# cherise215/Cooperative_Training_and_Latent_Space_Data_Augmentation

Measured on AMD Instinct MI355X. Metric: cooperative-training slices/sec (256x256, bs16 per GPU), higher is better.
Workload: dtype f32 (bf16x3 split)

## Files before the change

cooperative_training_and_latent_space_data_augmentation_amd/_ffi.py:

```python
from __future__ import annotations

import ctypes as C
import os

import numpy as np

_HERE = os.path.dirname(os.path.abspath(__file__))
LIB_PATH = os.path.join(_HERE, "csrc", "libctl_hip.so")
ABI_VERSION = 11
RED_BLOCKS = 512

IN_PLAIN, IN_UP2, IN_ZINS2, IN_C4 = 0, 1, 2, 3
ACT_NONE, ACT_LEAKY, ACT_SIGMOID = 0, 1, 2
EPI_BIAS, EPI_ACCUM, EPI_RES, EPI_STATS, EPI_BNBWD, EPI_TAILBWD = 1, 2, 4, 8, 16, 32
(OP_CONV, OP_WGRAD, OP_WGRAD_REDUCE, OP_PACK, OP_BN_FINALIZE, OP_BN_EVAL, OP_BN_ACT, OP_BWD_REDUCE, OP_BN_BWD_FINALIZE,
 OP_BWD_APPLY, OP_CHAN_SUM_FINALIZE, OP_SUMPOOL2, OP_SIGMOID_BWD, OP_ZERO, OP_COPY, OP_PACK_BATCH, OP_WGRAD_REDUCE_BATCH, OP_DROPOUT2D, OP_BN_REPLAY,
 OP_WGRAD_GROUP) = range(1, 21)
WGRAD_GROUP_MAX = 8
OP_MAX_T = 14

CONV_DTYPE = np.dtype([
    ("n", "<i4"), ("hin", "<i4"), ("win", "<i4"), ("cin", "<i4"), ("hout", "<i4"), ("wout", "<i4"), ("cout", "<i4"),
    ("ks", "<i4"), ("stride", "<i4"), ("pad", "<i4"), ("in_mode", "<i4"), ("pro_affine", "<i4"), ("pro_slope", "<f4"),
    ("epi_flags", "<i4"), ("epi_act", "<i4"), ("epi_slope", "<f4"), ("out_h", "<i4"), ("out_w", "<i4"),
    ("out_sy", "<i4"), ("out_sx", "<i4"), ("nsub", "<i4"), ("out_sub", "<i4"), ("groups", "<i4"), ("dt", "<i4")])
DT_BF16, DT_X16, DT_Y16, DT_RES16, DT_X3 = 1, 2, 4, 8, 16
PACK_X3 = 16
LOSS_WCE, LOSS_FOCAL, LOSS_DICE, LOSS_FG_DICE = 0, 1, 2, 3
OP_DTYPE = np.dtype([("kind", "<i4"), ("i", "<i4", (27,)), ("f", "<f4", (4,)), ("slot", "<i4", (OP_MAX_T,)),
                     ("off", "<i8", (OP_MAX_T,)), ("l", "<i8", (4,))], align=True)


class CtlError(RuntimeError):
    pass


class _Lib:
    def __init__(self):
        self._lib = None

    def load(self):
        if self._lib is not None:
            return self._lib
        if not os.path.exists(LIB_PATH):
            raise CtlError(f"HIP extension not built: {LIB_PATH} is missing. Run `python -c 'import __graft_entry__ as g; "
                           "g.build()'` (or `make -C <package>/csrc`). There is no fallback path.")
        import torch
        lib = C.CDLL(LIB_PATH)
        lib.ctl_last_error.restype = C.c_char_p
        lib.ctl_version.restype = C.c_int
        lib.ctl_launch_count.restype = C.c_ulonglong
        for name in ("ctl_conv_wpack_floats", "ctl_conv_stats_floats", "ctl_wgrad_partial_floats",
                     "ctl_wgrad_bias_partial_floats", "ctl_latent_score_ws_floats", "ctl_latent_mask_apply_ws_floats",
                     "ctl_rescale_intensity_ws_floats", "ctl_sizeof_op", "ctl_sizeof_conv", "ctl_latent_mask_fused_ws_floats", "ctl_conv_wpack_floats_x3",
                     "ctl_surface_stats_ws_bytes", "ctl_surface_map_ws_bytes", "ctl_cc_ws_bytes", "ctl_aug_ws_bytes", "ctl_aug_warp_ws_bytes",
                     "ctl_surface_quantiles_ws_bytes",
                     "ctl_aug_spline_ws_bytes", "ctl_aug_warp_cubic_ws_bytes", "ctl_aug_bias_ws_bytes", "ctl_order_stats_ws_bytes", "ctl_corrupt_spike_ws_bytes",
                     "ctl_seg_loss_ws_doubles"):
            getattr(lib, name).restype = C.c_size_t
        p, i32, i64, f32, u64 = C.c_void_p, C.c_int32, C.c_int64, C.c_float, C.c_uint64
        sig = {
            "ctl_conv_wpack_floats": [i32, i32, i32],
            "ctl_conv_stats_floats": [p], "ctl_conv_stats_blocks": [p],
            "ctl_wgrad_splits": [p], "ctl_wgrad_partial_floats": [p], "ctl_wgrad_bias_partial_floats": [p],
            "ctl_pack_weights": [p, p, i32, i32, i32, i64, i64, i64, i64, i32, p],
            "ctl_conv_forward": [p] * 12, "ctl_conv_forward_ex": [p] * 16, "ctl_conv_pool_ok": [p],
            "ctl_conv_wgrad": [p] * 8, "ctl_conv_wgrad_ex": [p] * 10,
            "ctl_wgrad_group_class": [p, i32], "ctl_wgrad_group_plan": [p, i32, p], "ctl_conv_wgrad_group": [i32] + [p] * 11,
            "ctl_wgrad_reduce": [p, p, p, p, i64, i64, i64, i64, p, i32, p],
            "ctl_confusion_hist": [p, p, i64, i32, p, p],
            "ctl_rescale_intensity": [p, p, p, i32, i64, f32, f32, f32, p],
            "ctl_noise_clamp": [p, p, u64, f32, f32, f32, p, i64, p],
            "ctl_rescale_intensity_ws_floats": [i32],
            "ctl_crop_or_pad": [p, p, i32, i32, i32, i32, i32, i32, p],
            "ctl_bn_finalize": [p, i32, i32, i64, p, p, f32, f32, i32, p, p, p, p, p, p, p, i32, p],
            "ctl_bn_finalize_ex": [p, i32, i32, i64, p, p, f32, f32, i32, p, p, p, p, p, p, p, p, i32, p],
            "ctl_bn_replay_running": [p, p, p, p, i32, f32, p],
            "ctl_bn_eval_coeffs": [i32, p, p, p, p, f32, p, p, i32, p],
            "ctl_bn_act": [p, p, p, f32, p, i64, i32, i32, p],
            "ctl_bwd_reduce": [i32, p, p, p, p, p, f32, i64, i32, p, i32, p], "ctl_red_blocks": [],
            "ctl_bn_bwd_finalize": [p, i32, i64, p, p, p, p, p, p, i32, i32, i32, p],
            "ctl_bn_bwd_finalize_ex": [p, i32, i64, p, p, p, p, p, p, i32, i32, i32, C.c_uint32, p],
            "ctl_bwd_apply": [i32, p, p, p, p, p, f32, p, i64, i32, p, p, i32, p],
            "ctl_chan_sum_finalize": [p, i32, p, i32, p],
            "ctl_sumpool2": [p, p, i32, i32, i32, i32, i32, p],
            "ctl_sigmoid_bwd": [p, p, p, i64, p],
            "ctl_softmax_t_fwd": [p, f32, p, i64, i32, p],
            "ctl_softmax_t_bwd": [p, p, f32, p, i64, i32, p],
            "ctl_onehot": [p, p, i64, i32, p],
            "ctl_ce2d_fwd": [p, p, i64, i32, p, p, p],
            "ctl_ce2d_bwd": [p, p, p, i64, i32, p, p],
            "ctl_mse_fwd": [p, p, i64, f32, p, p, p],
            "ctl_mse_bwd": [p, p, p, i64, f32, p, p],
            "ctl_argmax_c": [p, p, i64, i32, p],
            "ctl_latent_score_ws_floats": [i32, i32, i32, i32],
            "ctl_latent_score": [i32, p, p, p, i32, i32, i32, p],
            "ctl_latent_mask_apply": [i32, p, p, p, i32, p, p, p, p, i32, i32, i32, p],
            "ctl_latent_mask_apply_ws_floats": [i32, i32, i32, i32],
            "ctl_latent_mask_fused_ws_floats": [i32, i32, i32, i32],
            "ctl_latent_mask_fused": [i32, p, p, p, i32, p, p, p, p, p, i32, i32, i32, p],
            "ctl_dropout2d": [p, p, u64, f32, p, p, i32, i32, i32, p],
            "ctl_uniform": [p, i64, u64, p],
            "ctl_step_tick": [p, p],
            "ctl_spin": [i32, p],
            "ctl_dropout2d_ex": [p, p, u64, p, f32, p, p, p, i32, i32, i32, p],
            "ctl_dropout2d_dt": [p, p, u64, p, f32, p, p, i32, i32, i32, C.c_uint32, p],
            "ctl_uniform_dev": [p, i64, u64, p, p],
            "ctl_adam_dev": [p, p, p, p, i64, f32, f32, f32, f32, p, f32, p],
            "ctl_adam": [p, p, p, p, i64, f32, f32, f32, f32, i32, f32, p],
            "ctl_accumulate": [p, p, i32, i64, p],
            "ctl_plan_run": [p, i32, p, i32, p],
            "ctl_prof_start": [C.c_char_p], "ctl_prof_start_sampled": [C.c_char_p, i32], "ctl_prof_stop": [p, C.c_size_t],
            "ctl_pack_weights_batched": [p, p, p, i32, i64, p], "ctl_wgrad_reduce_batched": [p, p, p, i32, i64, p],
            "ctl_pack_weights_bf16_batched": [p, p, p, i32, i64, p],
            "ctl_pack_weights_x3_batched": [p, p, p, i32, i64, p], "ctl_conv_wpack_floats_x3": [i32, i32, i32],
            "ctl_bwd_reduce_rows": [i32, i64, i32],
            "ctl_bn_act_dt": [p, p, p, f32, p, i64, i32, i32, C.c_uint32, p],
            "ctl_bwd_reduce_dt": [i32, p, p, p, p, p, f32, i64, i32, p, i32, C.c_uint32, p, p],
            "ctl_bwd_apply_dt": [i32, p, p, p, p, p, f32, p, i64, i32, p, p, i32, C.c_uint32, p],
            "ctl_sumpool2_dt": [p, p, i32, i32, i32, i32, i32, C.c_uint32, p],
            "ctl_surface_stats_rows": [i32, i32, i32, i32], "ctl_surface_stats_ws_bytes": [i32] * 6,
            "ctl_surface_stats": [p, p, i32, i32, i32, i32, i32, i32, i32, p, p, p, C.c_size_t, p],
            "ctl_surface_map_ws_bytes": [i32] * 4,
            "ctl_surface_quantiles_ws_bytes": [i32] * 7,
            "ctl_surface_quantiles": [p, p, i32, i32, i32, i32, i32, i32, i32, p, p, i32, p, p, p, C.c_size_t, p],
            "ctl_surface_map": [p, i32, i32, i32, i32, i32, p, p, p, p, C.c_size_t, p],
            "ctl_cc_ws_bytes": [i32] * 5, "ctl_cc_label": [p, i32, i32, i32, i32, i32, i32, p, p],
            "ctl_cc_keep_largest": [p, i32, i32, i32, i32, i32, i32, p, p, p, C.c_size_t, p],
            "ctl_aug_ws_bytes": [i32] * 3, "ctl_aug_warp_ws_bytes": [i32] * 5, "ctl_aug_field": [p, p, p, p, i32, i32, i32, p, p, C.c_size_t, p],
            "ctl_aug_warp": [p, p, p, p, p, i32, i32, i32, i32, i32, p, p, p, C.c_size_t, p],
            "ctl_aug_spline_ws_bytes": [i32] * 4, "ctl_aug_warp_cubic_ws_bytes": [i32] * 6,
            "ctl_aug_spline_coeffs": [p, p, p, i32, i32, i32, i32, p, p, C.c_size_t, p],
            "ctl_aug_warp_cubic": [p, p, p, p, p, i32, i32, i32, i32, i32, i32, p, p, p, C.c_size_t, p],
            "ctl_aug_bias_ws_bytes": [i32] * 3, "ctl_aug_bias": [p, p, p, p, i32, i32, i32, p, p, C.c_size_t, p],
            "ctl_aug_coarse_field": [p, i32, i32, i32, p, p],
            "ctl_order_stats_ws_bytes": [i32, i32], "ctl_order_stats": [p, i32, i64, p, i32, p, p, C.c_size_t, p],
            "ctl_percentile_apply": [p, p, i32, i64, C.c_double, C.c_double, i32, f32, f32, p, p, p],
            "ctl_resample_inplane": [p, p, i32, i32, i32, i32, i32, i32, C.c_double, C.c_double, p, p, p],
            "ctl_restore_scores": [p, i32, i32, i32, i32, i32, i32, i32, i32, i32, i32, C.c_double, C.c_double, i32, p, p, p],
            "ctl_restore_labels": [p, i32, i32, i32, i32, i32, i32, i32, i32, i32, C.c_double, C.c_double, p, p],
            "ctl_corrupt_bias": [p, p, i32, i32, i32, p, p], "ctl_corrupt_spike_ws_bytes": [i32] * 4,
            "ctl_corrupt_spike": [p, i32, i32, i32, p, p, i32, C.c_double, p, p, C.c_size_t, p],
            "ctl_corrupt_rigid3d": [p, i32, i32, i32, p, i32, p, p], "ctl_axis_operator": [p, p, i32, i32, i32, i32, i32, p, p, p],
            "ctl_slice_foreground": [p, p, i32, i64, p, p],
            "ctl_batch_gather": [p, p, p, i32, i64, p, i32, p, i32, i32, p, p, i32, i32, p, p, p],
            "ctl_seg_loss_blocks": [i32, i64], "ctl_seg_loss_ws_doubles": [i32, i32, i64, i32],
            "ctl_seg_loss_fwd": [i32, p, p, p, f32, i32, i64, i32, p, p, p],
            "ctl_seg_loss_bwd": [i32, p, p, p, f32, p, p, i32, i64, i32, p, p],
        }
        for name, args in sig.items():
            getattr(lib, name).argtypes = args
        if lib.ctl_version() != ABI_VERSION or lib.ctl_sizeof_op() != OP_DTYPE.itemsize or lib.ctl_sizeof_conv() != CONV_DTYPE.itemsize:
            raise CtlError(f"ABI mismatch: library version {lib.ctl_version()} vs binding {ABI_VERSION}, sizeof(ctl_op)={lib.ctl_sizeof_op()} "
                           f"vs {OP_DTYPE.itemsize}, sizeof(ctl_conv)={lib.ctl_sizeof_conv()} vs {CONV_DTYPE.itemsize}")
        if lib.ctl_red_blocks() != RED_BLOCKS:
            raise CtlError(f"ABI mismatch: the library was built with CTL_RED_BLOCKS={lib.ctl_red_blocks()}, this binding sizes scratch for {RED_BLOCKS}")
        self._lib = lib
        return lib

    def __getattr__(self, name):
        return getattr(self.load(), name)


lib = _Lib()

EXPORTED = ["ctl_version", "ctl_last_error", "ctl_conv_wpack_floats", "ctl_conv_stats_floats", "ctl_conv_stats_blocks",
            "ctl_pack_weights", "ctl_conv_forward", "ctl_conv_forward_ex", "ctl_conv_pool_ok", "ctl_wgrad_splits", "ctl_wgrad_partial_floats",
            "ctl_wgrad_bias_partial_floats", "ctl_conv_wgrad", "ctl_conv_wgrad_ex", "ctl_wgrad_reduce", "ctl_bn_finalize", "ctl_bn_finalize_ex", "ctl_bn_replay_running", "ctl_bn_eval_coeffs",
            "ctl_bn_act", "ctl_bwd_reduce", "ctl_bn_bwd_finalize", "ctl_bn_bwd_finalize_ex", "ctl_bwd_apply", "ctl_chan_sum_finalize", "ctl_sumpool2",
            "ctl_sigmoid_bwd", "ctl_softmax_t_fwd", "ctl_softmax_t_bwd", "ctl_onehot", "ctl_ce2d_fwd", "ctl_ce2d_bwd",
            "ctl_mse_fwd", "ctl_mse_bwd", "ctl_argmax_c", "ctl_latent_score_ws_floats", "ctl_latent_score",
            "ctl_latent_mask_apply", "ctl_latent_mask_apply_ws_floats", "ctl_dropout2d", "ctl_uniform", "ctl_adam", "ctl_plan_run", "ctl_sizeof_op",
            "ctl_sizeof_conv", "ctl_prof_start", "ctl_prof_start_sampled", "ctl_prof_stop", "ctl_pack_weights_batched",
            "ctl_wgrad_reduce_batched", "ctl_confusion_hist", "ctl_rescale_intensity_ws_floats", "ctl_rescale_intensity",
            "ctl_noise_clamp", "ctl_crop_or_pad", "ctl_step_tick", "ctl_spin", "ctl_dropout2d_ex", "ctl_dropout2d_dt", "ctl_uniform_dev", "ctl_adam_dev",
            "ctl_latent_mask_fused_ws_floats", "ctl_latent_mask_fused", "ctl_accumulate", "ctl_pack_weights_bf16_batched",
            "ctl_bn_act_dt", "ctl_bwd_reduce_dt", "ctl_bwd_apply_dt", "ctl_sumpool2_dt", "ctl_bwd_reduce_rows", "ctl_red_blocks",
            "ctl_launch_count", "ctl_conv_wpack_floats_x3", "ctl_pack_weights_x3_batched", "ctl_wgrad_group_class", "ctl_wgrad_group_plan",
            "ctl_conv_wgrad_group", "ctl_surface_stats_rows", "ctl_surface_stats_ws_bytes", "ctl_surface_stats", "ctl_surface_map_ws_bytes",
            "ctl_surface_map", "ctl_cc_ws_bytes", "ctl_cc_label", "ctl_cc_keep_largest", "ctl_aug_ws_bytes", "ctl_aug_warp_ws_bytes", "ctl_aug_field",
            "ctl_aug_warp", "ctl_aug_spline_ws_bytes", "ctl_aug_warp_cubic_ws_bytes", "ctl_aug_spline_coeffs", "ctl_aug_warp_cubic",
            "ctl_aug_bias_ws_bytes", "ctl_aug_bias", "ctl_aug_coarse_field", "ctl_order_stats_ws_bytes", "ctl_order_stats",
            "ctl_percentile_apply", "ctl_resample_inplane", "ctl_corrupt_bias", "ctl_corrupt_spike_ws_bytes", "ctl_corrupt_spike",
            "ctl_corrupt_rigid3d", "ctl_axis_operator", "ctl_slice_foreground", "ctl_batch_gather", "ctl_surface_quantiles_ws_bytes",
            "ctl_surface_quantiles", "ctl_restore_scores", "ctl_restore_labels", "ctl_seg_loss_blocks", "ctl_seg_loss_ws_doubles",
            "ctl_seg_loss_fwd", "ctl_seg_loss_bwd"]


def prof_start(kernel_filter: str = "", every: int = 1) -> None:
    check(lib.ctl_prof_start_sampled(kernel_filter.encode(), int(every)), "ctl_prof_start_sampled")


def prof_stop() -> dict:
    buf = C.create_string_buffer(1 << 18)
    check(lib.ctl_prof_stop(buf, len(buf)), "ctl_prof_stop")
    out = {}
    for line in buf.value.decode().splitlines():
        parts = line.split()
        out[parts[0]] = {k: float(v) for k, v in (kv.split("=") for kv in parts[1:])}
    return out


def check(rc: int, what: str = "") -> None:
    if rc != 0:
        msg = lib.ctl_last_error()
        raise CtlError(f"{what} failed (rc={rc}): {msg.decode() if msg else ''}")


def conv_desc(**kw) -> np.ndarray:
    d = np.zeros((), dtype=CONV_DTYPE)
    d["pad"] = 1 if kw.get("ks", 3) in (3, 4) else 0
    d["stride"] = 1
    d["nsub"] = 1
    d["groups"] = 1
    d["out_sy"] = d["out_sx"] = 1
    for k, v in kw.items():
        d[k] = v
    if "out_h" not in kw:
        d["out_h"] = d["hout"]
    if "out_w" not in kw:
        d["out_w"] = d["wout"]
    return d


def desc_ptr(d: np.ndarray) -> int:
    return d.ctypes.data
```

cooperative_training_and_latent_space_data_augmentation_amd/csrc/ctl_conv.hip:

```cpp
#include <stdlib.h>

#include <type_traits>

#include "ctl_common.h"

#include "ctl_conv_common.h"

#ifdef CTL_TIMING
#define CTL_TM_WAVES 65536
__device__ unsigned long long ctl_tm[CTL_TM_WAVES][10];
#define TM_DECL unsigned long long tm_prev = __builtin_amdgcn_s_memtime(), tm_acc[10] = {0, 0, 0, 0, 0, 0, 0, 0, 0, 0}; \
                const unsigned long long tm_t0 = tm_prev, tm_r0 = __builtin_amdgcn_s_memrealtime();
#define TM(i) { const unsigned long long tm_now = __builtin_amdgcn_s_memtime(); tm_acc[i] += tm_now - tm_prev; tm_prev = tm_now; }
#define TM_COUNT(i) { tm_acc[i] += 1; }
#define TM_FLUSH { const unsigned w_ = ((blockIdx.x + gridDim.x * (blockIdx.y + gridDim.y * blockIdx.z)) * 4 + (threadIdx.x >> 6)) % CTL_TM_WAVES; \
                   tm_acc[8] = __builtin_amdgcn_s_memtime() - tm_t0; tm_acc[9] = __builtin_amdgcn_s_memrealtime() - tm_r0; \
                   if ((threadIdx.x & 63) == 0) { _Pragma("unroll") for (int i_ = 0; i_ < 10; ++i_) ctl_tm[w_][i_] += tm_acc[i_]; } }
extern "C" int ctl_debug_timing(unsigned long long* out8) {
    static unsigned long long host[CTL_TM_WAVES][10];
    if (hipMemcpyFromSymbol(host, HIP_SYMBOL(ctl_tm), sizeof(host)) != hipSuccess) return -1;
    for (int i = 0; i < 12; ++i) out8[i] = 0;
    for (int w = 0; w < CTL_TM_WAVES; ++w) {
        for (int i = 0; i < 10; ++i) out8[i] += host[w][i];
        if (host[w][8] > out8[10]) out8[10] = host[w][8];
// ... 540 lines not shown
    const bool is_w = idx < total;
    const bool is_b = !is_w && dbias != nullptr && idx < total + cout;
    float v = 0.f;
    int co = 0, ci = 0, tap = 0;
    if (is_w) {
        co = idx % cout;
        ci = (idx / cout) % cin;
        tap = idx / ((int64_t)cout * cin);
        const int64_t stride = (int64_t)taps * cin_p * cout_p;
        const float* src = w_partial + ((int64_t)tap * cin_p + ci) * cout_p + co;
        for (int s = sl; s < splits; s += 8) v += src[s * stride];
    } else if (is_b) {
        co = idx - total;
        for (int s = sl; s < splits; s += 8) v += b_partial[(int64_t)s * cout_p + co];
    }
    sm[sl][e] = v;
    __syncthreads();
    if (sl == 0 && (is_w || is_b)) {
        float t = 0.f;
#pragma unroll
        for (int k = 0; k < 8; ++k) t += sm[k][e];
        float* dst = is_w ? dw + co * s_co + ci * s_ci + (tap / ks) * s_kh + (tap % ks) * s_kw : dbias + co;
        *dst = accumulate ? (*dst + t) : t;
    }
}

__global__ void pack_weights_kernel(const float* __restrict__ src, float* __restrict__ dst, int cout, int cin, int ks,
                                    int g_chunks, int64_t total, int64_t s_co, int64_t s_ci, int64_t s_kh,
                                    int64_t s_kw, int flip) {
    const int64_t idx = (int64_t)blockIdx.x * blockDim.x + threadIdx.x;
    if (idx >= total) return;
    const int j = idx & 3, lane = (idx >> 2) & 63;
    int64_t rest = idx >> 8;
    const int g = rest % g_chunks;
    rest /= g_chunks;
    const int taps = ks * ks;
    const int tap = rest % taps;
    const int cot = rest / taps;
    const int co = cot * 16 + (lane & 15);
    const int ci = g * 16 + (lane >> 4) * 4 + j;
    int kh = tap / ks, kw = tap % ks;
    if (flip) { kh = ks - 1 - kh; kw = ks - 1 - kw; }
    float v = 0.f;
    if (co < cout && ci < cin) v = src[co * s_co + ci * s_ci + kh * s_kh + kw * s_kw];
    dst[idx] = v;
}

__global__ void pack_weights_batched_kernel(const float* __restrict__ params, float* __restrict__ wpack,
                                            const int64_t* __restrict__ table) {
    const int64_t* r = table + (int64_t)blockIdx.y * 12;
    const int64_t total = r[10];
    const int64_t idx = (int64_t)blockIdx.x * blockDim.x + threadIdx.x;
    if (idx >= total || (r[11] & CTL_PACK_X3)) return;
    const float* src = params + r[0];
    float* dst = wpack + r[1];
    const int cout = (int)r[2], cin = (int)r[3], ks = (int)r[4], flip = (int)r[5];
    const int g_chunks = (cin + 15) / 16;
    const int j = idx & 3, lane = (idx >> 2) & 63;
    int64_t rest = idx >> 8;
    const int g = rest % g_chunks;
    rest /= g_chunks;
    const int taps = ks * ks;
    const int tap = rest % taps;
    const int cot = rest / taps;
    const int co = cot * 16 + (lane & 15);
    const int ci = g * 16 + (lane >> 4) * 4 + j;
    int kh = tap / ks, kw = tap % ks;
    float v = 0.f;
    if (r[11] == 4) {
        const int c = j, quad = (int)((idx >> 8) % 3), cot4 = (int)((idx >> 8) / 3);
        const int co4 = cot4 * 16 + (lane & 15), tp = 4 * quad + (lane >> 4);
        if (co4 < cout && c < cin && tp < 9) v = src[co4 * r[6] + c * r[7] + (tp / 3) * r[8] + (tp % 3) * r[9]];
        dst[idx] = v;
        return;
    }
    if (r[11] == 1) {
        if (co < cout && ci < cin) {
            for (int a = 0; a < 2; ++a) {
                const int sh = a + 2 - kh;
                if (sh < 0 || sh > 2) continue;
                for (int b = 0; b < 2; ++b) {
                    const int sw = b + 2 - kw;
                    if (sw < 0 || sw > 2) continue;
                    v += src[co * r[6] + ci * r[7] + sh * r[8] + sw * r[9]];
                }
            }
        }
    } else if (r[11] == 2) {
        if (co < cout && ci < cin) {
            const int a = flip >> 1, b = flip & 1;
            const int h0 = (kh == 0) ? 0 : (a ? 2 : 1), h1 = (kh == 0) ? (a ? 1 : 0) : 2;
            const int w0 = (kw == 0) ? 0 : (b ? 2 : 1), w1 = (kw == 0) ? (b ? 1 : 0) : 2;
            for (int sh = h0; sh <= h1; ++sh)
                for (int sw = w0; sw <= w1; ++sw) v += src[co * r[6] + ci * r[7] + sh * r[8] + sw * r[9]];
        }
    } else if (r[11] == 3) {
        if (co < cout && ci < cin) {
            const int a = flip >> 1, b = flip & 1;
            const int sh = a ? (kh == 0 ? 2 : 0) : (kh == 0 ? 1 : -1);
            const int sw = b ? (kw == 0 ? 2 : 0) : (kw == 0 ? 1 : -1);
            if (sh >= 0 && sw >= 0) v = src[co * r[6] + ci * r[7] + sh * r[8] + sw * r[9]];
        }
    } else {
        if (flip) { kh = ks - 1 - kh; kw = ks - 1 - kw; }
        if (co < cout && ci < cin) v = src[co * r[6] + ci * r[7] + kh * r[8] + kw * r[9]];
    }
    dst[idx] = v;
}

__global__ __launch_bounds__(256) void wgrad_reduce_batched_kernel(const float* __restrict__ scratch, float* __restrict__ grad,
                                                                    const int64_t* __restrict__ table) {
    __shared__ float sm[32][65];
    const int64_t* r = table + (int64_t)blockIdx.y * 16;
    const int splits = (int)r[4], taps = (int)(r[5] & 0xff), ks = (int)(r[5] >> 8), cin = (int)r[6], cout = (int)r[7];
    const int cin_p = (int)r[8], cout_p = (int)r[9];
    const int64_t total = (int64_t)taps * cin * cout;
    const bool has_b = r[1] >= 0 && r[3] >= 0;
    const bool wide = splits <= 64;
    const int EW = wide ? 64 : 8, SLN = wide ? 4 : 32;
    if ((int64_t)blockIdx.x * EW >= total + (has_b ? cout : 0)) return;
    const int e = wide ? (threadIdx.x & 63) : (threadIdx.x & 7), sl = wide ? (threadIdx.x >> 6) : (threadIdx.x >> 3);
    const int64_t idx = (int64_t)blockIdx.x * EW + e;
    const bool is_w = idx < total, is_b = !is_w && has_b && idx < total + cout;
    float v = 0.f;
    int co = 0, ci = 0, tap = 0;
    if (is_w) {
        co = idx % cout;
        ci = (idx / cout) % cin;
        tap = idx / ((int64_t)cout * cin);
        const int64_t stride = (int64_t)taps * cin_p * cout_p;
        const float* src = scratch + r[0] + ((int64_t)tap * cin_p + ci) * cout_p + co;
        for (int s0 = sl; s0 < splits; s0 += 8 * SLN) {
            float t8[8];
#pragma unroll
            for (int u = 0; u < 8; ++u) { const int s = s0 + u * SLN; t8[u] = s < splits ? src[s * stride] : 0.f; }
#pragma unroll
            for (int u = 0; u < 8; ++u) v += t8[u];
        }
    } else if (is_b) {
        co = idx - total;
        const float* src = scratch + r[1] + co;
        for (int s = sl; s < splits; s += SLN) v += src[(int64_t)s * cout_p];
    }
    sm[sl][e] = v;
    __syncthreads();
    if (sl == 0 && (is_w || is_b)) {
        float t = 0.f;
        for (int k = 0; k < SLN; ++k) t += sm[k][e];
        float* dst = is_w ? grad + r[2] + co * r[10] + ci * r[11] + (tap / ks) * r[12] + (tap % ks) * r[13] : grad + r[3] + co;
        *dst = r[14] ? (*dst + t) : t;
    }
}

extern "C" int ctl_pack_weights_batched(const float* params, float* wpack, const int64_t* table, int32_t n_rec,
                                        int64_t max_total, ctl_stream stream) {
    CTL_REQUIRE(params && wpack && table && n_rec > 0 && max_total > 0, "pack_weights_batched: bad arguments");
    pack_weights_batched_kernel<<<dim3((unsigned)ctl_cdiv64(max_total, 256), (unsigned)n_rec), dim3(256), 0, (hipStream_t)stream>>>(
        params, wpack, table);
    CTL_LAUNCH_CHECK("pack_weights_batched");
    return CTL_OK;
}
extern "C" int ctl_wgrad_reduce_batched(const float* scratch, float* grad, const int64_t* table, int32_t n_rec,
                                        int64_t max_elems, ctl_stream stream) {
    CTL_REQUIRE(scratch && grad && table && n_rec > 0 && max_elems > 0, "wgrad_reduce_batched: bad arguments");
    wgrad_reduce_batched_kernel<<<dim3((unsigned)max_elems, (unsigned)n_rec), dim3(256), 0, (hipStream_t)stream>>>(
        scratch, grad, table);
    CTL_LAUNCH_CHECK("wgrad_reduce_batched");
    return CTL_OK;
}

extern "C" size_t ctl_conv_wpack_floats(int32_t cin, int32_t cout, int32_t ks) {
    return (size_t)ctl_cdiv(cout, 16) * ks * ks * ctl_cdiv(cin, 16) * 256;
}

static bool conv_combo_ok(const ctl_conv* d) {
    const int k = d->ks, s = d->stride, m = d->in_mode, pd = d->pad;
    if (k == 3 && s == 1 && pd == 1 && m != CTL_IN_C4) return true;
    if (k == 3 && s == 1 && pd == 1 && m == CTL_IN_C4 && d->cin <= 4 && d->nsub == 1) return true;
    if (k == 3 && s == 2 && pd == 1 && m == CTL_IN_PLAIN) return true;
    if (k == 1 && s == 1 && pd == 0 && m != CTL_IN_ZINS2) return true;
    if (k == 2 && s == 2 && pd == 0 && m == CTL_IN_PLAIN) return true;
    if (k == 4 && s == 2 && pd == 1 && m == CTL_IN_PLAIN) return true;
    if (k == 2 && s == 1 && (pd == 0 || pd == 2) && m == CTL_IN_PLAIN && d->nsub == 4) return true;
    return false;
}

int ctl_conv_pick_cfg(const ctl_conv* d, ctl_conv_cfg* c, int for_wgrad) {
    CTL_REQUIRE(conv_combo_ok(d), "conv: unsupported ks/stride/pad/in_mode %d/%d/%d/%d", d->ks, d->stride, d->pad,
                d->in_mode);
    CTL_REQUIRE(d->cin == 1 || d->cin % 4 == 0, "conv: cin must be 1 or a multiple of 4 (got %d)", d->cin);
    CTL_REQUIRE(d->cout == 1 || d->cout % 4 == 0, "conv: cout must be 1 or a multiple of 4 (got %d)", d->cout);
    CTL_REQUIRE(d->cin < 16 ? (d->cin == 1 || d->cin == 4 || d->cin == 8 || d->cin == 12) : d->cin % 16 == 0,
                "conv: cin >= 16 must be a multiple of 16 (got %d)", d->cin);
    CTL_REQUIRE(d->nsub == 1 || d->nsub == 4, "conv: nsub must be 1 or 4");
    c->cot = ctl_cdiv(d->cout, 16);
    c->g = ctl_cdiv(d->cin, 16);
    c->nt = (c->cot % 2 == 0) ? 2 : 1;
    auto blocks = [&](int mt, int tw) {
        const int th = 4 * mt * 16 / tw;
        return (int64_t)d->n * ctl_cdiv(d->hout, th) * ctl_cdiv(d->wout, tw) * (c->cot / c->nt) * d->nsub;
    };
    int mt, tw;
    if (for_wgrad) {
        if (d->hout >= 8) { mt = 2; tw = 16; }
        else { mt = 1; tw = 16; }
    } else if (d->stride == 2) {
        if (blocks(2, 16) >= 384) { mt = 2; tw = 16; } else { mt = 1; tw = 16; }
        if (d->ks == 4 && c->nt == 2) { mt = 1; tw = 16; }
    } else if (d->wout >= 32 && blocks(4, 32) >= 512 && !(c->nt == 2 && blocks(4, 32) > 768)) {
        mt = 4; tw = 32;
    } else if (blocks(2, 16) >= 384) {
        mt = 2; tw = 16;
// ... 390 lines not shown
```

cooperative_training_and_latent_space_data_augmentation_amd/csrc/ctl_conv_common.h:

```cpp
#pragma once
#include "ctl_common.h"

template <int KS, int S, int MT, int TW>
struct Geom {
    static constexpr int MTILES = 4 * MT;
    static constexpr int TH = MTILES * 16 / TW;
    static constexpr int TP = TH * TW;
    static constexpr int IH = (TH - 1) * S + KS;
    static constexpr int IW = (TW - 1) * S + KS;
    static constexpr int IWH = (IW + 1) / 2;
    static constexpr int IWP = (S == 2) ? 2 * IWH : IW;
    static constexpr int XT_IMAGE = IH * IWP * 16;
    static constexpr int XT_FLOATS = XT_IMAGE + 4;
    static constexpr int PAD = (KS >= 3) ? 1 : 0;
    __device__ static __forceinline__ int ldscol(int c) { return (S == 2) ? ((c & 1) * IWH + (c >> 1)) : c; }
};

typedef unsigned int u32x4 __attribute__((ext_vector_type(4)));
#define CTL_OOB ((int)0x80000000)
#define CTL_PRO_MAX 256

__device__ __forceinline__ __amdgpu_buffer_rsrc_t ctl_rsrc(const void* p, int64_t bytes) {
    return __builtin_amdgcn_make_buffer_rsrc(const_cast<void*>(p), 0, (int)bytes, 0x00020000);
}
__device__ __forceinline__ f32x4 ctl_bload4(__amdgpu_buffer_rsrc_t r, int voff) {
    return __builtin_bit_cast(f32x4, __builtin_amdgcn_raw_buffer_load_b128(r, voff, 0, 0));
}
__device__ __forceinline__ float ctl_bload1(__amdgpu_buffer_rsrc_t r, int voff) {
    return __builtin_bit_cast(float, __builtin_amdgcn_raw_buffer_load_b32(r, voff, 0, 0));
}
#ifndef CTL_STORE_AUX
#define CTL_STORE_AUX 0
#endif
__device__ __forceinline__ void ctl_bstore4(__amdgpu_buffer_rsrc_t r, int voff, f32x4 v) {
    __builtin_amdgcn_raw_buffer_store_b128(__builtin_bit_cast(u32x4, v), r, voff, 0, CTL_STORE_AUX);
}
__device__ __forceinline__ void ctl_bstore1(__amdgpu_buffer_rsrc_t r, int voff, float v) {
    __builtin_amdgcn_raw_buffer_store_b32(__builtin_bit_cast(unsigned int, v), r, voff, 0, 0);
}
__device__ __forceinline__ f32x4 ctl_bload4s(__amdgpu_buffer_rsrc_t r, int voff, int soff) {
    return __builtin_bit_cast(f32x4, __builtin_amdgcn_raw_buffer_load_b128(r, voff, soff, 0));
}
__device__ __forceinline__ f32x4 ctl_leaky01(f32x4 v, float slope) {
    const f32x4 m = v * slope;
    return f32x4{fmaxf(v.x, m.x), fmaxf(v.y, m.y), fmaxf(v.z, m.z), fmaxf(v.w, m.w)};
}

struct TileWalk {
    int n, th, tw;
    int dn, dth, dtw;
    int tiles_h, tiles_w;
    __device__ __forceinline__ void init(int bid0, int nblk, int tiles_h_, int tiles_w_) {
        tiles_h = tiles_h_; tiles_w = tiles_w_;
        tw = bid0 % tiles_w; int b = bid0 / tiles_w; th = b % tiles_h; n = b / tiles_h;
        dtw = nblk % tiles_w; b = nblk / tiles_w; dth = b % tiles_h; dn = b / tiles_h;
    }
    __device__ __forceinline__ void next() {
        tw += dtw;
        if (tw >= tiles_w) { tw -= tiles_w; ++th; }
        th += dth;
        if (th >= tiles_h) { th -= tiles_h; ++n; }
        n += dn;
    }
};
```

cooperative_training_and_latent_space_data_augmentation_amd/csrc/ctl_conv_x3.hip:

```cpp
#include "ctl_common.h"
#ifdef CTL_TIMING_X3
#define CTL_TM_WAVES 65536
__device__ unsigned long long ctl_tm3[CTL_TM_WAVES][10];
#define TM_DECL unsigned long long tm_prev = __builtin_amdgcn_s_memtime(), tm_acc[10] = {0, 0, 0, 0, 0, 0, 0, 0, 0, 0}; \
                const unsigned long long tm_t0 = tm_prev, tm_r0 = __builtin_amdgcn_s_memrealtime();
#define TM(i) { const unsigned long long tm_now = __builtin_amdgcn_s_memtime(); tm_acc[i] += tm_now - tm_prev; tm_prev = tm_now; }
#define TM_COUNT(i) { tm_acc[i] += 1; }
#ifdef CTL_TIMING_X3_VMCNT
#define CTL_TM3_REAL
#else
#define CTL_TM3_REAL tm_acc[9] = __builtin_amdgcn_s_memrealtime() - tm_r0;
#endif
#define TM_FLUSH { const unsigned w_ = ((blockIdx.x + gridDim.x * (blockIdx.y + gridDim.y * blockIdx.z)) * 8 + (threadIdx.x >> 6)) % CTL_TM_WAVES; \
                   tm_acc[8] = __builtin_amdgcn_s_memtime() - tm_t0; CTL_TM3_REAL \
                   if ((threadIdx.x & 63) == 0) { _Pragma("unroll") for (int i_ = 0; i_ < 10; ++i_) ctl_tm3[w_][i_] += tm_acc[i_]; } }
extern "C" int ctl_debug_timing_x3(unsigned long long* out12) {
    static unsigned long long host[CTL_TM_WAVES][10];
    if (hipMemcpyFromSymbol(host, HIP_SYMBOL(ctl_tm3), sizeof(host)) != hipSuccess) return -1;
    for (int i = 0; i < 12; ++i) out12[i] = 0;
    for (int w = 0; w < CTL_TM_WAVES; ++w) {
        for (int i = 0; i < 10; ++i) out12[i] += host[w][i];
        if (host[w][8] > out12[10]) out12[10] = host[w][8];
        if (host[w][8]) out12[11] += 1;
    }
    for (int w = 0; w < CTL_TM_WAVES; ++w) for (int i = 0; i < 10; ++i) host[w][i] = 0;
    return hipMemcpyToSymbol(HIP_SYMBOL(ctl_tm3), host, sizeof(host)) == hipSuccess ? 0 : -1;
}
#endif
#include "ctl_conv_igemm.h"

__device__ static float x3_pack_value(const float* __restrict__ src, const int64_t* __restrict__ r, int mode, int co, int ci, int kh, int kw) {
    const int cout = (int)r[2], cin = (int)r[3], ks = (int)r[4], flip = (int)r[5];
    if (co >= cout || ci >= cin) return 0.f;
    float v = 0.f;
    if (mode == 1) {
        for (int a = 0; a < 2; ++a) {
            const int sh = a + 2 - kh;
            if (sh < 0 || sh > 2) continue;
            for (int b = 0; b < 2; ++b) {
                const int sw = b + 2 - kw;
                if (sw < 0 || sw > 2) continue;
                v += src[co * r[6] + ci * r[7] + sh * r[8] + sw * r[9]];
            }
        }
    } else if (mode == 2) {
        const int a = flip >> 1, b = flip & 1;
        const int h0 = (kh == 0) ? 0 : (a ? 2 : 1), h1 = (kh == 0) ? (a ? 1 : 0) : 2;
        const int w0 = (kw == 0) ? 0 : (b ? 2 : 1), w1 = (kw == 0) ? (b ? 1 : 0) : 2;
        for (int sh = h0; sh <= h1; ++sh)
            for (int sw = w0; sw <= w1; ++sw) v += src[co * r[6] + ci * r[7] + sh * r[8] + sw * r[9]];
    } else if (mode == 3) {
        const int a = flip >> 1, b = flip & 1;
        const int sh = a ? (kh == 0 ? 2 : 0) : (kh == 0 ? 1 : -1);
        const int sw = b ? (kw == 0 ? 2 : 0) : (kw == 0 ? 1 : -1);
        if (sh >= 0 && sw >= 0) v = src[co * r[6] + ci * r[7] + sh * r[8] + sw * r[9]];
    } else {
        if (flip) { kh = ks - 1 - kh; kw = ks - 1 - kw; }
        v = src[co * r[6] + ci * r[7] + kh * r[8] + kw * r[9]];
    }
    return v;
}
__global__ void pack_weights_x3_batched_kernel(const float* __restrict__ params, float* __restrict__ wpack, const int64_t* __restrict__ table) {
    const int64_t* r = table + (int64_t)blockIdx.y * 12;
    if (!(r[11] & CTL_PACK_X3)) return;
    const int mode = (int)(r[11] & ~(int64_t)CTL_PACK_X3);
    const int cout = (int)r[2], cin = (int)r[3], ks = (int)r[4];
    const int g_chunks = (cin + 15) / 16, taps = ks * ks, nfrag = (taps + 1) / 2;
    const int64_t total = (int64_t)((cout + 15) / 16) * nfrag * g_chunks * 64 * 4;
    const int64_t idx = (int64_t)blockIdx.x * blockDim.x + threadIdx.x;
    if (idx >= total) return;
    const float* src = params + r[0];
    unsigned* dst = reinterpret_cast<unsigned*>(wpack + r[1]);
    const int jp = idx & 3, lane = (idx >> 2) & 63;
    int64_t rest = idx >> 8;
    const int g = rest % g_chunks;
    rest /= g_chunks;
    const int f = rest % nfrag;
    const int cot = rest / nfrag;
    const int co = cot * 16 + (lane & 15), q = lane >> 4;
    const int tap = 2 * f + (q >> 1);
    float a = 0.f, b = 0.f;
    if (tap < taps) {
        const int ci = g * 16 + (q & 1) * 8 + jp * 2;
        a = x3_pack_value(src, r, mode, co, ci, tap / ks, tap % ks);
        b = x3_pack_value(src, r, mode, co, ci + 1, tap / ks, tap % ks);
    }
    const int64_t base = ((((int64_t)cot * nfrag + f) * g_chunks + g) * 3) * 256 + lane * 4 + jp;
#pragma unroll
    for (int sp = 0; sp < 3; ++sp) dst[base + sp * 256] = x3_pack2(x3_part(a, sp), x3_part(b, sp));
}
extern "C" size_t ctl_conv_wpack_floats_x3(int32_t cin, int32_t cout, int32_t ks) {
    return (size_t)ctl_cdiv(cout, 16) * ((ks * ks + 1) / 2) * ctl_cdiv(cin, 16) * 3 * 256;
}
extern "C" int ctl_pack_weights_x3_batched(const float* params, float* wpack, const int64_t* table, int32_t n_rec, int64_t max_total, ctl_stream stream) {
    CTL_REQUIRE(params && wpack && table && n_rec > 0 && max_total > 0, "pack_weights_x3_batched: bad arguments");
    pack_weights_x3_batched_kernel<<<dim3((unsigned)ctl_cdiv64(max_total, 3 * 256) + 1, (unsigned)n_rec), dim3(256), 0, (hipStream_t)stream>>>(params, wpack, table);
    CTL_LAUNCH_CHECK("pack_weights_x3_batched");
    return CTL_OK;
}

struct conv3_call {
    const ctl_conv* d; ctl_conv_cfg c;
    const float *x, *wpack, *bias, *pro_scale, *pro_shift, *res, *res_scale, *res_shift, *res2, *x2;
    float *y, *stats_partial, *pool, *xout;
    hipStream_t stream;
    bool query;
    int grid_x;
    int stat_rows_per_block;
};

#ifndef CTL_X3_PC_DEFAULT
#define CTL_X3_PC_DEFAULT 1
#endif
#ifndef CTL_X3_PC_MIN_STEPS
#define CTL_X3_PC_MIN_STEPS 4
#endif
static bool conv3_pc_shape_ok(const ctl_conv* d) {
    const int f = d->epi_flags & (CTL_EPI_RES | CTL_EPI_ACCUM | CTL_EPI_BNBWD | CTL_EPI_TAILBWD);
    const bool epi_ok = f == 0 || (f == CTL_EPI_BNBWD && d->cout % 16 == 0 && d->epi_act == CTL_ACT_NONE);
    return d->ks == 3 && d->stride == 1 && d->in_mode == CTL_IN_PLAIN && d->nsub == 1 && epi_ok;
}
template <int KS, int S, int MODE, int MT, int TW, int NT, int EPI, bool X2>
constexpr bool conv3_pc_ok() { return S == 1 && KS == 3 && MODE == CTL_IN_PLAIN && (EPI == 0 || EPI == 3); }
template <int KS, int S, int MODE, int MT, int TW, int NT, int EPI, bool X2>
static bool conv3_go_pc(conv3_call& a) {
    if constexpr (conv3_pc_ok<KS, S, MODE, MT, TW, NT, EPI, X2>()) {
        if (!a.c.pc) return false;
        const ctl_conv* d = a.d;
        const int ntiles = d->n * a.c.tiles_h * a.c.tiles_w;
        const int grid_x = ctl_conv_grid_x(ntiles, (a.c.cot / NT) * d->nsub, 1);
        a.grid_x = grid_x;
        a.stat_rows_per_block = 4;
        if (a.query) return true;
        const dim3 grid((unsigned)grid_x, (unsigned)(a.c.cot / NT), (unsigned)d->nsub);
        conv_igemm_kernel<KS, S, MODE, MT, TW, NT, EPI, X2, true, true><<<grid, dim3(512), 0, a.stream>>>(
            *d, a.x, a.wpack, a.bias, a.pro_scale, a.pro_shift, a.res, a.res_scale, a.res_shift, a.y, a.stats_partial, a.c.tiles_h,
            a.c.tiles_w, a.c.g, (int64_t)ctl_conv_wpack_floats_x3(d->cin, d->cout, d->ks), ntiles, a.res2, a.x2, a.pool, a.xout);
        return true;
    }
    return false;
}
template <int KS, int S, int MODE, int MT, int TW, int NT, int EPI, bool X2 = false>
static void conv3_go(conv3_call& a) {
    if constexpr (!X2 && ((KS == 3 && S == 1 && MODE == CTL_IN_PLAIN) || (KS == 4 && S == 2)) && EPI != 2) {
        if (a.d->pro_affine == 2) { conv3_go<KS, S, MODE, MT, TW, NT, EPI, true>(a); return; }
    }
    a.stat_rows_per_block = 1;
    if (conv3_go_pc<KS, S, MODE, MT, TW, NT, EPI, X2>(a)) return;
    static int occ = 0;
    if (!occ) {
// ... 128 lines not shown
```

cooperative_training_and_latent_space_data_augmentation_amd/csrc/ctl_elem.hip:

```cpp
#include "ctl_common.h"

#define EB 256
#ifndef CTL_FIN_THREADS
#define CTL_FIN_THREADS EB
#endif
#define MAX_STREAM_BLOCKS 2048

static inline unsigned stream_blocks(int64_t work_items) {
    int64_t b = ctl_cdiv64(work_items, EB);
    if (b > MAX_STREAM_BLOCKS) b = MAX_STREAM_BLOCKS;
    if (b < 1) b = 1;
    return (unsigned)b;
}

__device__ __forceinline__ void block_sum_double2(double& a, double& b, double* sm) {
    for (int o = 32; o > 0; o >>= 1) { a += __shfl_xor(a, o); b += __shfl_xor(b, o); }
    const int w = threadIdx.x >> 6;
    if ((threadIdx.x & 63) == 0) { sm[w] = a; sm[8 + w] = b; }
    __syncthreads();
    if (threadIdx.x == 0) {
        a = b = 0.0;
        for (int i = 0; i < (int)(blockDim.x >> 6); ++i) { a += sm[i]; b += sm[8 + i]; }
    }
    __syncthreads();
// ... 511 lines not shown
                                                       float* __restrict__ dlogit) {
    const int c = CT ? CT : c_rt;
    const float gs = gout[0] / (float)pixels;
    const int64_t stride = (int64_t)gridDim.x * EB;
    for (int64_t i = (int64_t)blockIdx.x * EB + threadIdx.x; i < pixels; i += stride) {
        float v[CT ? CT : MAXC];
        row_load<CT>(logit, i, c, v);
        float m = -INFINITY;
#pragma unroll
        for (int k = 0; k < c; ++k) m = fmaxf(m, v[k]);
        float s = 0.f;
#pragma unroll
        for (int k = 0; k < c; ++k) { v[k] = expf(v[k] - m); s += v[k]; }
        const float r = 1.f / s;
        const int l = (int)label[i];
#pragma unroll
        for (int k = 0; k < c; ++k) v[k] = gs * (v[k] * r - ((k == l) ? 1.f : 0.f));
        row_store<CT>(dlogit, i, c, v);
    }
}
__global__ __launch_bounds__(EB) void mse_partial_kernel(const float* __restrict__ a, const float* __restrict__ b,
                                                          int64_t count, double* __restrict__ partial) {
    __shared__ double sm[8];
    const int64_t stride = (int64_t)gridDim.x * EB;
    double acc = 0.0;
    for (int64_t i = (int64_t)blockIdx.x * EB + threadIdx.x; i < count; i += stride) {
        const float d = a[i] - b[i];
        acc += (double)(d * d);
    }
    acc = block_sum_double(acc, sm);
    if (threadIdx.x == 0) partial[blockIdx.x] = acc;
}
__global__ __launch_bounds__(EB) void mse_bwd_kernel(const float* __restrict__ a, const float* __restrict__ b,
                                                      const float* __restrict__ gout, int64_t count, float scale,
                                                      float* __restrict__ da) {
    const float gs = gout[0] * 2.f * scale / (float)count;
    const int64_t stride = (int64_t)gridDim.x * EB;
    for (int64_t i = (int64_t)blockIdx.x * EB + threadIdx.x; i < count; i += stride) da[i] = gs * (a[i] - b[i]);
}
__global__ __launch_bounds__(EB) void argmax_kernel(const float* __restrict__ logit, uint8_t* __restrict__ out,
                                                     int64_t pixels, int c) {
    const int64_t stride = (int64_t)gridDim.x * EB;
    for (int64_t i = (int64_t)blockIdx.x * EB + threadIdx.x; i < pixels; i += stride) {
        float best = logit[i * c];
        int bi = 0;
        for (int k = 1; k < c; ++k) {
            const float v = logit[i * c + k];
            if (v > best) { best = v; bi = k; }
        }
        out[i] = (uint8_t)bi;
    }
}

__global__ __launch_bounds__(EB) void adam_kernel(float* __restrict__ p, const float* __restrict__ g, float* __restrict__ m,
                                                   float* __restrict__ v, int64_t count, float lr, float b1, float b2,
                                                   float eps, float bc1, float bc2_sqrt, float gscale,
                                                   const int64_t* __restrict__ state) {
    if (state) {
        const double st = (double)state[2];
        bc1 = (float)(1.0 - pow((double)b1, st));
        bc2_sqrt = (float)sqrt(1.0 - pow((double)b2, st));
    }
    const int64_t stride = (int64_t)gridDim.x * EB;
    const float step_size = lr / bc1;
    for (int64_t i = (int64_t)blockIdx.x * EB + threadIdx.x; i < count; i += stride) {
        const float gi = g[i] * gscale;
        const float mi = b1 * m[i] + (1.f - b1) * gi;
        const float vi = b2 * v[i] + (1.f - b2) * gi * gi;
        m[i] = mi;
        v[i] = vi;
        const float denom = sqrtf(vi) / bc2_sqrt + eps;
        p[i] = p[i] - step_size * (mi / denom);
    }
}

struct ctl_ptr8 { const float* p[8]; };
__global__ __launch_bounds__(EB) void accumulate_kernel(float* __restrict__ dst, ctl_ptr8 src, int k, int64_t count) {
    const int64_t stride = (int64_t)gridDim.x * EB;
    for (int64_t i = (int64_t)blockIdx.x * EB + threadIdx.x; i < count; i += stride) {
        float a = dst[i];
        for (int j = 0; j < k; ++j) a += src.p[j][i];
        dst[i] = a;
    }
}

#define S_ (hipStream_t) stream

extern "C" int ctl_accumulate(float* dst, const float* const* srcs, int32_t k, int64_t count, ctl_stream stream) {
    CTL_REQUIRE(dst && srcs && k >= 1 && k <= 8 && count > 0, "accumulate: bad arguments (1 <= k <= 8)");
    ctl_ptr8 a;
    for (int j = 0; j < 8; ++j) a.p[j] = j < k ? srcs[j] : nullptr;
    for (int j = 0; j < k; ++j) CTL_REQUIRE(a.p[j], "accumulate: null source %d", j);
    accumulate_kernel<<<dim3(stream_blocks(count)), dim3(EB), 0, S_>>>(dst, a, k, count);
    CTL_LAUNCH_CHECK("accumulate");
    return CTL_OK;
}

__global__ void bn_replay_running_kernel(const char* __restrict__ act, float* __restrict__ buffers, int64_t* __restrict__ nbt,
                                         const int64_t* __restrict__ table, float momentum) {
    const int64_t* r = table + (int64_t)blockIdx.x * 6;
    const float* mean = reinterpret_cast<const float*>(act + r[0]);
    const float* uvar = reinterpret_cast<const float*>(act + r[1]);
    float* rm = buffers + r[2];
    float* rv = buffers + r[3];
    const int c = (int)r[5];
    for (int ch = threadIdx.x; ch < c; ch += blockDim.x) {
        rm[ch] = (1.f - momentum) * rm[ch] + momentum * mean[ch];
        rv[ch] = (1.f - momentum) * rv[ch] + momentum * uvar[ch];
    }
    if (threadIdx.x == 0) nbt[r[4]] += 1;
}
extern "C" int ctl_bn_replay_running(const void* act, float* buffers, int64_t* nbt, const int64_t* table, int32_t n_rec, float momentum,
                                     ctl_stream stream) {
    CTL_REQUIRE(act && buffers && nbt && table && n_rec > 0, "bn_replay_running: bad arguments");
    bn_replay_running_kernel<<<dim3((unsigned)n_rec), dim3(128), 0, (hipStream_t)stream>>>((const char*)act, buffers, nbt, table, momentum);
    CTL_LAUNCH_CHECK("bn_replay_running");
    return CTL_OK;
}
// ... 181 lines not shown
    return CTL_OK;
}
extern "C" int ctl_softmax_t_bwd(const float* p, const float* dp, float inv_t, float* dx, int64_t pixels, int32_t c,
                                 ctl_stream stream) {
    CTL_REQUIRE(p && dp && dx && pixels > 0 && c > 0 && c <= MAXC, "softmax_t_bwd: bad arguments");
    CTL_ROW_DISPATCH(softmax_t_bwd_kernel, rows_vec4(c, p, dp, dx), dim3(stream_blocks(pixels)), p, dp, inv_t, dx, pixels, c);
    CTL_LAUNCH_CHECK("softmax_t_bwd");
    return CTL_OK;
}
extern "C" int ctl_onehot(const int64_t* label, float* y, int64_t pixels, int32_t c, ctl_stream stream) {
    CTL_REQUIRE(label && y && pixels > 0 && c > 0, "onehot: bad arguments");
    onehot_kernel<<<dim3(stream_blocks(pixels)), dim3(EB), 0, S_>>>(label, y, pixels, c);
    CTL_LAUNCH_CHECK("onehot");
    return CTL_OK;
}
extern "C" int ctl_ce2d_fwd(const float* logit, const int64_t* label, int64_t pixels, int32_t c, double* partial,
                            float* loss, ctl_stream stream) {
    CTL_REQUIRE(logit && label && partial && loss && pixels > 0 && c > 0 && c <= MAXC, "ce2d_fwd: bad arguments");
    CTL_ROW_DISPATCH(ce2d_partial_kernel, rows_vec4(c, logit), dim3(CTL_RED_BLOCKS), logit, label, pixels, c, partial);
    scalar_finalize_kernel<<<dim3(1), dim3(EB), 0, S_>>>(partial, CTL_RED_BLOCKS, 1.0 / (double)pixels, loss);
    ctl_count_launches(1);
    CTL_LAUNCH_CHECK("ce2d_fwd");
    return CTL_OK;
}
extern "C" int ctl_ce2d_bwd(const float* logit, const int64_t* label, const float* gout, int64_t pixels, int32_t c,
                            float* dlogit, ctl_stream stream) {
    CTL_REQUIRE(logit && label && gout && dlogit && pixels > 0 && c > 0 && c <= MAXC, "ce2d_bwd: bad arguments");
    CTL_ROW_DISPATCH(ce2d_bwd_kernel, rows_vec4(c, logit, dlogit), dim3(stream_blocks(pixels)), logit, label, gout, pixels, c, dlogit);
    CTL_LAUNCH_CHECK("ce2d_bwd");
    return CTL_OK;
}
extern "C" int ctl_mse_fwd(const float* a, const float* b, int64_t count, float scale, double* partial, float* loss,
                           ctl_stream stream) {
    CTL_REQUIRE(a && b && partial && loss && count > 0, "mse_fwd: bad arguments");
    mse_partial_kernel<<<dim3(CTL_RED_BLOCKS), dim3(EB), 0, S_>>>(a, b, count, partial);
    scalar_finalize_kernel<<<dim3(1), dim3(EB), 0, S_>>>(partial, CTL_RED_BLOCKS, (double)scale / (double)count, loss);
    ctl_count_launches(1);
    CTL_LAUNCH_CHECK("mse_fwd");
    return CTL_OK;
}
extern "C" int ctl_mse_bwd(const float* a, const float* b, const float* gout, int64_t count, float scale, float* da,
                           ctl_stream stream) {
    CTL_REQUIRE(a && b && gout && da && count > 0, "mse_bwd: bad arguments");
    mse_bwd_kernel<<<dim3(stream_blocks(count)), dim3(EB), 0, S_>>>(a, b, gout, count, scale, da);
    CTL_LAUNCH_CHECK("mse_bwd");
    return CTL_OK;
}
extern "C" int ctl_argmax_c(const float* logit, uint8_t* out, int64_t pixels, int32_t c, ctl_stream stream) {
    CTL_REQUIRE(logit && out && pixels > 0 && c > 0 && c < 256, "argmax_c: bad arguments");
    argmax_kernel<<<dim3(stream_blocks(pixels)), dim3(EB), 0, S_>>>(logit, out, pixels, c);
    CTL_LAUNCH_CHECK("argmax_c");
    return CTL_OK;
}
extern "C" int ctl_adam(float* p, const float* g, float* m, float* v, int64_t count, float lr, float beta1, float beta2,
                        float eps, int32_t step, float grad_scale, ctl_stream stream) {
    CTL_REQUIRE(p && g && m && v && count > 0 && step >= 1, "adam: bad arguments");
    const double bc1 = 1.0 - pow((double)beta1, (double)step);
    const double bc2 = 1.0 - pow((double)beta2, (double)step);
    adam_kernel<<<dim3(stream_blocks(count)), dim3(EB), 0, S_>>>(p, g, m, v, count, lr, beta1, beta2, eps, (float)bc1,
                                                                 (float)sqrt(bc2), grad_scale, nullptr);
    CTL_LAUNCH_CHECK("adam");
    return CTL_OK;
}
extern "C" int ctl_adam_dev(float* p, const float* g, float* m, float* v, int64_t count, float lr, float beta1, float beta2,
                            float eps, const int64_t* state, float grad_scale, ctl_stream stream) {
    CTL_REQUIRE(p && g && m && v && count > 0 && state, "adam_dev: bad arguments");
    adam_kernel<<<dim3(stream_blocks(count)), dim3(EB), 0, S_>>>(p, g, m, v, count, lr, beta1, beta2, eps, 1.f, 1.f, grad_scale, state);
    CTL_LAUNCH_CHECK("adam_dev");
    return CTL_OK;
}
```

cooperative_training_and_latent_space_data_augmentation_amd/csrc/ctl_plan.cpp:

```cpp
#include <stdarg.h>
#include <stdlib.h>
#include <string.h>

#include "ctl_common.h"

static thread_local char g_err[512] = "";

void ctl_set_error(const char* fmt, ...) {
    va_list ap;
    va_start(ap, fmt);
    vsnprintf(g_err, sizeof(g_err), fmt, ap);
    va_end(ap);
}

#include <atomic>
#include <map>
#include <string>
#include <vector>
namespace {
struct ProfRec { std::string id; hipEvent_t a, b; double flops, bytes; void* stream; };
bool g_prof_on = false;
std::string g_prof_filter;
std::vector<ProfRec> g_prof;
std::vector<hipEvent_t> g_prof_pool;
// ... 233 lines not shown
                break;
            }
            case CTL_OP_WGRAD_REDUCE:
                memcpy(&d, op.i, sizeof(d));
                rc = ctl_wgrad_reduce(&d, CF(0), CF(1), F(2), op.l[0], op.l[1], op.l[2], op.l[3], F(3), op.i[24], stream);
                break;
            case CTL_OP_PACK:
                rc = ctl_pack_weights(CF(0), F(1), op.i[0], op.i[1], op.i[2], op.l[0], op.l[1], op.l[2], op.l[3], op.i[3], stream);
                break;
            case CTL_OP_BN_FINALIZE:
                rc = ctl_bn_finalize_ex(CF(0), op.i[0], op.i[1], op.l[0], CF(1), CF(2), op.f[0], op.f[1], op.i[2], F(3), F(4),
                                        (int64_t*)t[5], F(6), F(7), F(8), F(9), F(10), NG(op.i[3]), stream);
                break;
            case CTL_OP_BN_REPLAY:
                rc = ctl_bn_replay_running(t[0], F(1), (int64_t*)t[2], (const int64_t*)t[3], op.i[0], op.f[0], stream);
                break;
            case CTL_OP_BN_EVAL:
                rc = ctl_bn_eval_coeffs(op.i[0], CF(0), CF(1), CF(2), CF(3), op.f[0], F(4), F(5), NG(op.i[1]), stream);
                break;
            case CTL_OP_BN_ACT:
                rc = ctl_bn_act_dt(CF(0), CF(1), CF(2), op.f[0], F(3), op.l[0], op.i[0], NG(op.i[1]), (uint32_t)op.i[25], stream);
                break;
            case CTL_OP_BWD_REDUCE:
                rc = ctl_bwd_reduce_dt(op.i[0], CF(0), CF(1), CF(2), CF(3), CF(4), op.f[0], op.l[0], op.i[1], F(5), NG(op.i[2]), (uint32_t)op.i[25], F(6), stream);
                break;
            case CTL_OP_BN_BWD_FINALIZE:
                rc = ctl_bn_bwd_finalize_ex(CF(0), op.i[0], op.l[0], CF(1), CF(2), CF(3), F(4), F(5), F(6), op.i[1], NG(op.i[2]), op.i[3], (uint32_t)op.i[4], stream);
                break;
            case CTL_OP_BWD_APPLY:
                rc = ctl_bwd_apply_dt(op.i[0], CF(0), CF(1), CF(2), CF(3), CF(4), op.f[0], CF(5), op.l[0], op.i[1], F(6), F(7), NG(op.i[2]), (uint32_t)op.i[25], stream);
                break;
            case CTL_OP_CHAN_SUM_FINALIZE:
                rc = ctl_chan_sum_finalize(CF(0), op.i[0], F(1), op.i[1], stream);
                break;
            case CTL_OP_SUMPOOL2:
                rc = ctl_sumpool2_dt(CF(0), F(1), op.i[0], op.i[1], op.i[2], op.i[3], op.i[4], (uint32_t)op.i[25], stream);
                break;
            case CTL_OP_SIGMOID_BWD:
                rc = ctl_sigmoid_bwd(CF(0), CF(1), F(2), op.l[0], stream);
                break;
            case CTL_OP_ZERO: {
                CTL_REQUIRE(t[0] && op.l[0] > 0, "plan_run: op %d ZERO needs a pointer and a size", k);
                ctl_count_launches(1);
                hipError_t e = hipMemsetAsync(t[0], 0, (size_t)op.l[0], (hipStream_t)stream);
                if (e != hipSuccess) CTL_FAIL(CTL_ELAUNCH, "plan_run: memset: %s", hipGetErrorString(e));
                break;
            }
            case CTL_OP_PACK_BATCH:
                rc = (op.i[1] & 1) ? ctl_pack_weights_bf16_batched(CF(0), F(1), (const int64_t*)t[2], op.i[0], op.l[0], stream)
                                   : ctl_pack_weights_batched(CF(0), F(1), (const int64_t*)t[2], op.i[0], op.l[0], stream);
                if (rc == CTL_OK && (op.i[1] & 2)) rc = ctl_pack_weights_x3_batched(CF(0), F(1), (const int64_t*)t[2], op.i[0], op.l[0], stream);
                break;
            case CTL_OP_WGRAD_REDUCE_BATCH:
                rc = ctl_wgrad_reduce_batched(CF(0), F(1), (const int64_t*)t[2], op.i[0], op.l[0], stream);
                break;
            case CTL_OP_DROPOUT2D:
                rc = ctl_dropout2d_dt(t[0], CF(1), (uint64_t)op.l[0], (const int64_t*)t[2], op.f[0], t[3], F(4), op.i[0], op.i[1], op.i[2], (uint32_t)op.i[25], stream);
                break;
            case CTL_OP_COPY: {
                CTL_REQUIRE(t[0] && t[1] && op.l[0] > 0, "plan_run: op %d COPY needs two pointers and a size", k);
                ctl_count_launches(1);
                hipError_t e = hipMemcpyAsync(t[1], t[0], (size_t)op.l[0], hipMemcpyDeviceToDevice, (hipStream_t)stream);
                if (e != hipSuccess) CTL_FAIL(CTL_ELAUNCH, "plan_run: memcpy: %s", hipGetErrorString(e));
                break;
            }
            default:
                CTL_FAIL(CTL_EINVAL, "plan_run: op %d has unknown kind %d", k, op.kind);
        }
#undef F
#undef CF
#undef NG
        if (ptok >= 0) ctl_prof_end(ptok, (hipStream_t)stream);
        if (rc != CTL_OK) {
            char msg[400];
            snprintf(msg, sizeof(msg), "%s", g_err);
            ctl_set_error("plan_run: op %d (kind %d) failed: %s", k, op.kind, msg);
            return rc;
        }
    }
    return CTL_OK;
}
```

cooperative_training_and_latent_space_data_augmentation_amd/nets.py:

```python
from __future__ import annotations

import ctypes
from collections import namedtuple
from typing import Dict, List, Optional, Tuple

import numpy as np
import torch
import torch.nn as nn

from . import _ffi, init as _init
from ._ffi import lib, check, OP_DTYPE

(S_X, S_P, S_B, S_NBT, S_WP, S_ACT, S_SCR, S_OUT0, S_OUT1, S_DOUT0, S_DOUT1, S_GRAD, S_DX, S_BSCR, S_TAB, S_STATE, S_KEEP) = range(17)
N_SLOTS = 17
SLOPE = 0.2
EPS = 1e-5
MOMENTUM = 0.1
SMALL_CIN = True
PHASE_CONVS = True
FUSE_BNBWD = True
FUSE_BNAPPLY = True
FUSE_BNBWD16 = True
FUSE_XOUT16 = True
FUSE_XOUT = False
# ... 128 lines not shown
        self.rec, self.groups = rec, groups


class PassStack:

    def __init__(self, net: "CtlNet", P: int = 2):
        self.net, self.P = net, P
        self.lease = None
        self.outs = None
        self.shape = None
        self.plans, self.modes, self.xs, self.roots, self.need_dx, self.seqs = [], [], [], [], [], []
        self.douts = []
        self.keep = []
        self.events = []
        self.done = False

    @property
    def filled(self) -> int:
        return len(self.plans)

    def accepts(self, n, h, w, groups) -> bool:
        return (not self.done and self.filled < self.P and self.net.drop_p is None and
                (self.shape is None or self.shape == (n, h, w, groups)))

    def receive(self, p: int, douts):
        cur = self.douts[p]
        for k, d in enumerate(douts):
            if d is None:
                continue
            d = d.float().contiguous(memory_format=torch.channels_last)
            cur[k] = d if cur[k] is None else cur[k] + d
        ev = torch.cuda.Event()
        ev.record()
        self.events[p].append(ev)


class PlanBuilder:
    def __init__(self, net: "CtlNet"):
        self.net = net
        self.groups = int(getattr(net, "_cur_groups", 1))
        self.ops: List[np.ndarray] = []
        self.b16 = bool(getattr(net, "bf16", False))
        self.pp = tuple(getattr(net, "_cur_pp", (0, 1)))
        self.affine_mask = int(getattr(net, "_cur_affine_mask", 0))
        self.split_tail = bool(getattr(net, "_cur_split", False))
        self.act = Arena(S_ACT, self.b16, self.pp)
        self.bscr = Arena(S_BSCR, self.b16)
        self.scr_bytes = 0
        self.reduce_recs: List[list] = []
        self.pending_wgrads: List[dict] = []
        self.table: Optional[np.ndarray] = None
        self.bn_log: List[tuple] = []
        self.pro_entries = 0

    def op(self, kind: int) -> np.ndarray:
        r = np.zeros((), dtype=OP_DTYPE)
        r["kind"] = kind
        r["slot"][:] = -1
        self.ops.append(r)
        return r

    @staticmethod
    def set_t(op, idx, ref):
        if ref is not None:
            op["slot"][idx] = ref[0]
            op["off"][idx] = ref[1]

    def scr(self, *nbytes):
        refs, off = [], 0
        for nb in nbytes:
            refs.append((S_SCR, off))
            off += _rup(int(nb), 256)
        self.scr_bytes = max(self.scr_bytes, off)
        return refs

    @staticmethod
    def P(off_floats):
        return (S_P, 4 * off_floats)

    @staticmethod
    def G(off_floats):
        return (S_GRAD, 4 * off_floats)

    def _conv_desc(self, x: T, cout, ks, stride, in_mode, hout, wout, pro, flags, act, slope, nsub=1, pad=None, dt=0):
        d = _ffi.conv_desc(n=x.n, hin=x.h, win=x.w, cin=x.c, hout=hout, wout=wout, cout=cout, ks=ks, stride=stride,
                           pad=(1 if ks in (3, 4) else 0) if pad is None else pad, in_mode=in_mode, pro_affine=1 if pro else 0,
                           pro_slope=pro[2] if pro else 0.0, epi_flags=flags, epi_act=act, epi_slope=slope, dt=dt)
        if nsub == 4:
            d["out_h"], d["out_w"], d["out_sy"], d["out_sx"], d["nsub"], d["out_sub"] = 2 * hout, 2 * wout, 2, 2, 4, 1
        d["groups"] = self.groups
        if pro:
            self.pro_entries = max(self.pro_entries, self.groups * x.c)
        return d

    def conv(self, x: T, wp_ref, cout, ks, *, stride=1, in_mode=0, pro=None, bias_ref=None, stats=False, act=0,
             slope=0.0, res=None, accum=False, out: Optional[T] = None, arena: Optional[Arena] = None, nsub=1,
             hout=None, wout=None, bnbwd=None, pad=None, tail=None, x2=None, keep_stats=False, xout: Optional[T] = None):
        res2, want_pool, pool_t = None, False, None
        if tail is not None:
            assert res is None and bnbwd is None and bias_ref is None and act == 0
            stats, res2, slope = True, tail[1], tail[2]
            want_pool = len(tail) > 3 and bool(tail[3])
        if bnbwd is not None:
            assert res is None and not accum and bias_ref is None and act == 0
            stats, res, slope = True, (bnbwd[0], bnbwd[1], bnbwd[2]), bnbwd[3]
        if hout is None:
# ... 36 lines not shown
            else:
                stats_ref, = self.scr(4 * self.groups * blocks * 2 * cout)
        for idx, ref in enumerate([x.ref, wp_ref, bias_ref, pro[0] if pro else None, pro[1] if pro else None,
                                   (tail[0].ref if tail is not None else (res[0].ref if res else None)), res[1] if res else None, res[2] if res else None,
                                   out.ref, stats_ref, res2.ref if res2 is not None else None, x2[0].ref if x2 is not None else None,
                                   pool_t.ref if pool_t is not None else None, xout.ref if xout is not None else None]):
            self.set_t(op, idx, ref)
        assert xout is None or (x2 is not None and (xout.n, xout.h, xout.w, xout.c, xout.b16) == (x.n, x.h, x.w, x.c, x.b16))
        return out, stats_ref, blocks

    def wgrad(self, x: T, dy: T, ks, *, stride=1, in_mode=0, pro=None, dw_ref, strides, dbias_ref=None, accumulate=False, dy2=None):
        assert dy2 is None or (dy.b16 == dy2[0].b16 == self.b16 and ks == 3 and stride == 1)
        dt = (_ffi.DT_BF16 | (_ffi.DT_X16 if x.b16 else 0) | (_ffi.DT_Y16 if dy.b16 else 0)) if self.b16 else 0
        if (X3 and X3_WGRAD and not self.b16 and x.c % 16 == 0 and dy.c % 16 == 0 and
                ((ks == 3 and in_mode in (_ffi.IN_PLAIN, _ffi.IN_UP2) and (stride == 1 or in_mode == _ffi.IN_PLAIN)) or (ks == 2 and stride == 2 and in_mode == _ffi.IN_PLAIN))):
            dt = _ffi.DT_X3
        d = self._conv_desc(x, dy.c, ks, stride, in_mode, dy.h, dy.w, pro, 0, 0, 0.0, dt=dt)
        dp = _ffi.desc_ptr(d)
        assert dw_ref[0] == S_GRAD and (dbias_ref is None or dbias_ref[0] == S_GRAD)
        refs = [x.ref, pro[0] if pro else None, pro[1] if pro else None, dy.ref, None, None, dy2[0].ref if dy2 else None, dy2[1] if dy2 else None]
        if GROUP_WGRAD and (dt == _ffi.DT_X3 or (GROUP_WGRAD_BF16 and self.b16)):
            cls = int(lib.ctl_wgrad_group_class(dp, 1 if dy2 else 0))
            if cls >= 0:
                self.pending_wgrads.append(dict(cls=cls, d=d, refs=refs, dw_ref=dw_ref, dbias_ref=dbias_ref, strides=[int(v) for v in strides],
                                                accumulate=bool(accumulate), cin=x.c, cout=dy.c, ks=ks))
                return
        self._emit_wgrad(d, refs, dw_ref, dbias_ref, strides, accumulate, x.c, dy.c, ks, None)

    def _emit_wgrad(self, d, refs, dw_ref, dbias_ref, strides, accumulate, cin, cout, ks, splits):
        dp = _ffi.desc_ptr(d)
        cin_p, cout_p = _rup(cin, 16), _rup(cout, 16)
        if splits is None:
            wb, bb = 4 * lib.ctl_wgrad_partial_floats(dp), 4 * lib.ctl_wgrad_bias_partial_floats(dp)
        else:
            wb, bb = 4 * splits * ks * ks * cin_p * cout_p, 4 * splits * cout_p
        if wb == 0:
            raise _ffi.CtlError("wgrad plan: " + lib.ctl_last_error().decode())
        wref = self.bscr.alloc(wb)
        bref = self.bscr.alloc(bb) if dbias_ref is not None else None
        words = np.frombuffer(d.tobytes(), dtype="<i4")
        op = self.op(_ffi.OP_WGRAD)
        op["i"][:CONV_WORDS] = words
        refs = list(refs)
        refs[4], refs[5] = wref, bref
        for idx, ref in enumerate(refs):
            self.set_t(op, idx, ref)
        if splits is None:
            splits = lib.ctl_wgrad_splits(dp)
        else:
            op["i"][CONV_WORDS] = splits
        self.reduce_recs.append([wref[1] // 4, bref[1] // 4 if bref else -1, dw_ref[1] // 4, dbias_ref[1] // 4 if dbias_ref else -1,
                                 splits, (ks * ks) | (ks << 8), cin, cout, cin_p, cout_p, *[int(v) for v in strides],
                                 1 if accumulate else 0, 0])

    def flush_wgrad_groups(self):
        pend, self.pending_wgrads = self.pending_wgrads, []
        by_cls: Dict[int, list] = {}
        for w in pend:
            by_cls.setdefault(w["cls"], []).append(w)
        for cls in sorted(by_cls):
            members = by_cls[cls]
            for g0 in range(0, len(members), _ffi.WGRAD_GROUP_MAX):
                grp = members[g0:g0 + _ffi.WGRAD_GROUP_MAX]
                if len(grp) == 1:
                    w = grp[0]
                    self._emit_wgrad(w["d"], w["refs"], w["dw_ref"], w["dbias_ref"], w["strides"], w["accumulate"], w["cin"], w["cout"], w["ks"], None)
                    continue
                descs = np.concatenate([np.atleast_1d(w["d"]) for w in grp])
                splits = np.zeros(len(grp), dtype=np.int32)
                _ffi.check(lib.ctl_wgrad_group_plan(descs.ctypes.data, len(grp), splits.ctypes.data), "ctl_wgrad_group_plan")
                op = self.op(_ffi.OP_WGRAD_GROUP)
                op["i"][0] = len(grp)
                for w, sp in zip(grp, splits):
                    self._emit_wgrad(w["d"], w["refs"], w["dw_ref"], w["dbias_ref"], w["strides"], w["accumulate"], w["cin"], w["cout"], w["ks"], int(sp))

    def flush_wgrad_reductions(self):
        self.flush_wgrad_groups()
        if not self.reduce_recs:
            return
        assert self.table is None
        self.table = np.asarray(self.reduce_recs, dtype=np.int64)
        op = self.op(_ffi.OP_WGRAD_REDUCE_BATCH)
        op["i"][0] = len(self.reduce_recs)
        op["l"][0] = max(-(-((r[5] & 0xff) * r[6] * r[7] + r[7]) // (64 if r[4] <= 64 else 8)) for r in self.reduce_recs)
        self.set_t(op, 0, (S_BSCR, 0))
        self.set_t(op, 1, (S_GRAD, 0))
        self.set_t(op, 2, (S_TAB, 0))
        self.reduce_recs = []

    def bn_forward(self, bn: BNInfo, stats_ref, blocks, count, mode: str):
        c, G = bn.c, self.groups
        assert count % G == 0
        count //= G
        co = {k: self.act.rows(c, G) for k in ("scale", "shift", "mean", "invstd", "uvar")}
        if mode == "C":
            op = self.op(_ffi.OP_BN_EVAL)
            op["i"][0], op["i"][1] = c, G
            op["f"][0] = EPS
            for idx, ref in enumerate([self.P(bn.g_off), self.P(bn.b_off), (S_B, 4 * bn.rm_off), (S_B, 4 * bn.rv_off),
                                       co["scale"], co["shift"]]):
                self.set_t(op, idx, ref)
            return co
        op = self.op(_ffi.OP_BN_FINALIZE)
        op["i"][0], op["i"][1], op["i"][2], op["i"][3] = blocks, c, 1 if mode == "A" else 0, G
        op["l"][0] = count
        op["f"][0], op["f"][1] = EPS, MOMENTUM
        for idx, ref in enumerate([stats_ref, self.P(bn.g_off), self.P(bn.b_off), (S_B, 4 * bn.rm_off),
                                   (S_B, 4 * bn.rv_off), (S_NBT, 8 * bn.nbt_idx), co["scale"], co["shift"], co["mean"],
                                   co["invstd"], co["uvar"]]):
            self.set_t(op, idx, ref)
        self.bn_log.append((bn, co))
        return co

    @staticmethod
    def mask(*ts) -> int:
        return sum(1 << k for k, t in enumerate(ts) if t is not None and t.b16)

    def bn_act(self, x: T, co, slope, out: T):
        op = self.op(_ffi.OP_BN_ACT)
        op["i"][0], op["i"][1] = x.c, self.groups
        op["i"][25] = self.mask(x, out)
        op["l"][0] = x.n * x.h * x.w
        op["f"][0] = slope
        for idx, ref in enumerate([x.ref, co["scale"], co["shift"], out.ref]):
            self.set_t(op, idx, ref)

    def bn_backward(self, mode_kind: int, dy: T, act_src: Optional[T], bn_src: T, bn: BNInfo, co, slope, *, ds: Optional[T],
                    dx: T, affine_grad: bool):
        c, pixels, G = bn_src.c, bn_src.n * bn_src.h * bn_src.w, self.groups
        assert dx is not None or (mode_kind == 0 and ds is not None)
        part, = self.scr(4 * G * _ffi.RED_BLOCKS * 2 * c)
        coef = self.bscr.alloc(4 * 3 * c * G)
        ds_early = mode_kind == 0 and ds is not None and (not self.b16 or dx is None)
        op = self.op(_ffi.OP_BWD_REDUCE)
        op["i"][0], op["i"][1], op["i"][2] = mode_kind, c, G
        op["i"][25] = self.mask(dy, act_src, bn_src, ds if ds_early else None)
        op["l"][0] = pixels
        op["f"][0] = slope
        for idx, ref in enumerate([dy.ref, act_src.ref if act_src else None, bn_src.ref, co["scale"], co["shift"], part,
                                   ds.ref if ds_early else None]):
            self.set_t(op, idx, ref)
        op = self.op(_ffi.OP_BN_BWD_FINALIZE)
        op["i"][0], op["i"][1], op["i"][2], op["i"][4] = c, 0, G, self.affine_mask
        op["l"][0] = pixels // G
        for idx, ref in enumerate([part, self.P(bn.g_off), co["mean"], co["invstd"], coef,
                                   self.G(bn.g_off) if affine_grad else None, self.G(bn.b_off) if affine_grad else None]):
            self.set_t(op, idx, ref)
        if dx is None:
            return coef
        op = self.op(_ffi.OP_BWD_APPLY)
        if ds_early:
            op["i"][0], op["i"][1], op["i"][2] = 2, c, G
            op["i"][25] = self.mask(ds, None, bn_src, None, dx)
            op["l"][0] = pixels
            for idx, ref in enumerate([ds.ref, None, bn_src.ref, None, None, coef, None, dx.ref]):
                self.set_t(op, idx, ref)
            return coef
        op["i"][0], op["i"][1], op["i"][2] = mode_kind, c, G
        op["i"][25] = self.mask(dy, act_src, bn_src, ds, dx)
        op["l"][0] = pixels
        op["f"][0] = slope
        for idx, ref in enumerate([dy.ref, act_src.ref if act_src else None, bn_src.ref, co["scale"], co["shift"], coef,
                                   ds.ref if ds else None, dx.ref]):
            self.set_t(op, idx, ref)
        return coef

    def bn_backward_from_stats(self, g: T, bn_src: T, bn: BNInfo, co, stats_ref, blocks, *, dx: T, affine_grad: bool):
        c, pixels, G = bn_src.c, bn_src.n * bn_src.h * bn_src.w, self.groups
        coef = self.bscr.alloc(4 * 3 * c * G)
        op = self.op(_ffi.OP_BN_BWD_FINALIZE)
        op["i"][0], op["i"][1], op["i"][2], op["i"][3], op["i"][4] = c, 0, G, blocks, self.affine_mask
        op["l"][0] = pixels // G
        for idx, ref in enumerate([stats_ref, self.P(bn.g_off), co["mean"], co["invstd"], coef,
                                   self.G(bn.g_off) if affine_grad else None, self.G(bn.b_off) if affine_grad else None]):
            self.set_t(op, idx, ref)
        if dx is None:
            return coef
        op = self.op(_ffi.OP_BWD_APPLY)
        op["i"][0], op["i"][1], op["i"][2] = 2, c, G
        op["i"][25] = self.mask(g, None, bn_src, None, dx)
        op["l"][0] = pixels
        for idx, ref in enumerate([g.ref, None, bn_src.ref, None, None, coef, None, dx.ref]):
            self.set_t(op, idx, ref)
        return coef

    def chan_sum(self, dy: T, out_ref):
        c = dy.c
        part, = self.scr(4 * _ffi.RED_BLOCKS * 2 * c)
        op = self.op(_ffi.OP_BWD_REDUCE)
        op["i"][0], op["i"][1] = 2, c
        op["i"][25] = self.mask(dy)
        op["l"][0] = dy.n * dy.h * dy.w
        self.set_t(op, 0, dy.ref)
        self.set_t(op, 5, part)
        op = self.op(_ffi.OP_CHAN_SUM_FINALIZE)
        op["i"][0], op["i"][1] = c, 0
        self.set_t(op, 0, part)
        self.set_t(op, 1, out_ref)

    def sumpool2(self, dup: T, dx: T, accumulate=False):
        op = self.op(_ffi.OP_SUMPOOL2)
        op["i"][:5] = [dx.n, dx.h, dx.w, dx.c, 1 if accumulate else 0]
        op["i"][25] = self.mask(dup, dx)
        self.set_t(op, 0, dup.ref)
        self.set_t(op, 1, dx.ref)

    def sigmoid_bwd(self, dy: T, y: T, dx: T):
        assert not (dy.b16 or y.b16 or dx.b16), "sigmoid_bwd works on the fp32 network output"
        op = self.op(_ffi.OP_SIGMOID_BWD)
        op["l"][0] = y.n * y.h * y.w * y.c
        for idx, ref in enumerate([dy.ref, y.ref, dx.ref]):
            self.set_t(op, idx, ref)

    def dropout(self, z: T, out: T, p: float, *, keep_in=None, keep_out=None, salt: int = 0):
        op = self.op(_ffi.OP_DROPOUT2D)
        op["i"][25] = self.mask(z, out)
        op["i"][0], op["i"][1], op["i"][2] = z.n, z.h * z.w, z.c
        op["f"][0] = p
        op["l"][0] = salt
        for idx, ref in enumerate([z.ref, keep_in, None if keep_in is not None else (S_STATE, 0), out.ref, keep_out]):
            self.set_t(op, idx, ref)

    def zero(self, ref, nbytes):
        op = self.op(_ffi.OP_ZERO)
        op["l"][0] = nbytes
        self.set_t(op, 0, ref)

    def copy(self, src_ref, dst_ref, nbytes):
        op = self.op(_ffi.OP_COPY)
        op["l"][0] = nbytes
        self.set_t(op, 0, src_ref)
        self.set_t(op, 1, dst_ref)

    def finish(self, rec=None, out_shapes=None) -> Plan:
        self.flush_wgrad_reductions()
        p = Plan()
        p.replay = None
        p.table_np, p.table_dev = self.table, None
        p.ops = np.stack(self.ops) if self.ops else np.zeros(0, dtype=OP_DTYPE)
        p.ops = np.ascontiguousarray(p.ops)
        p.n_ops = len(self.ops)
        p.main_ops = p.tail_ops = None
        if self.split_tail:
            tail = []
            for k, o in enumerate(self.ops):
                kind = int(o["kind"])
                if kind in _TAIL_KINDS:
                    tail.append(k)
                    if kind == _ffi.OP_CHAN_SUM_FINALIZE:
                        assert int(self.ops[k - 1]["kind"]) == _ffi.OP_BWD_REDUCE and int(self.ops[k - 1]["i"][0]) == 2
                        tail.insert(len(tail) - 1, k - 1)
            ts = set(tail)
            main = [k for k in range(len(self.ops)) if k not in ts]
            p.main_ops = np.ascontiguousarray(p.ops[main])
            p.tail_ops = np.ascontiguousarray(p.ops[tail]) if tail else None
        p.act_bytes, p.scr_bytes, p.bscr_bytes = self.act.size, self.scr_bytes, self.bscr.size
        p.rec, p.out_shapes = rec, out_shapes
        p.groups = self.groups
        p.bn_log = self.bn_log
        p.pro_entries = self.pro_entries
        return p


class CtlNet(nn.Module):

    def __init__(self, spec, cin: int, device, bf16: bool = False):
        super().__init__()
        self._spec = spec
        self.cin = cin
        self.bf16 = bool(bf16)
        self._bn_track = True
        self._convs: Dict[str, ConvInfo] = {}
        self._bns: Dict[str, BNInfo] = {}
        self._plans: Dict[tuple, Plan] = {}
# ... 634 lines not shown
            ev = torch.cuda.Event()
            ev.record()
            self._deferred.append((seq, gflat, ev))
        else:
            self._flat.grad.add_(gflat)
            self._grad_written, self._grad_is_zero = True, False

    def _run_backward_stacked(self, stack: PassStack, x, douts, need_dx: bool, need_w: bool, tail_stream=None):
        P = stack.P
        n, h, w, G = stack.shape
        plan0 = stack.plans[0]
        mask = tuple(d is not None for d in douts)
        full = (1 << (P * G)) - 1
        amask = sum((((1 << G) - 1) << (p * G)) for p in range(P) if stack.modes[p] == "A")
        key = ("bs", n, h, w, tuple(stack.modes), mask, need_dx, need_w, P, G, id(plan0))
        plan = self._plans.get(key)
        if plan is None:
            view = _StackedForward(_stack_rec(plan0.rec, P), P * G)
            self._cur_groups, self._cur_affine_mask, self._cur_split = P * G, (0 if amask == full else amask), True
            try:
                plan = self._plans[key] = self._compile_backward(view, "A", mask, need_dx, need_w, amask != 0)
            finally:
                self._cur_groups, self._cur_affine_mask, self._cur_split = 1, 0, False
        lease = self._arenas.acquire(plan.bscr_bytes, self.device)
        stack.keep.append(lease)
        self._dbg_last = (plan, lease.t)
        tensors = {S_X: x, S_P: self._flat_data, S_WP: self._wp, S_ACT: stack.lease.t, S_BSCR: lease.t, S_OUT0: stack.outs[0]}
        if len(stack.outs) > 1:
            tensors[S_OUT1] = stack.outs[1]
        for slot, d in zip((S_DOUT0, S_DOUT1), douts):
            if d is not None:
                tensors[slot] = d
        dx = gflat = None
        if need_dx:
            dx = self._alloc_out((P * n, h, w, self.cin))
            tensors[S_DX] = dx
        if need_w:
            gflat = torch.empty(self._pcount, dtype=torch.float32, device=self.device)
            tensors[S_GRAD] = gflat
            self._grad_written, self._grad_is_zero = True, False
        if tail_stream is None or plan.tail_ops is None or not need_w:
            self._run(plan, tensors)
            return dx, gflat
        self._run(plan, tensors, ops=plan.main_ops)
        done = torch.cuda.Event()
        done.record()
        with torch.cuda.stream(tail_stream):
            tail_stream.wait_event(done)
            for t in tensors.values():
                t.record_stream(tail_stream)
            self._run(plan, tensors, ops=plan.tail_ops)
        return dx, gflat

    def run_backward(self, x, act, outs, fwd_plan: Plan, mode: str, douts, need_dx: bool, need_w: bool, affine: bool):
        n, c, h, w = x.shape
        mask = tuple(d is not None for d in douts)
        key = ("b", n, h, w, mode, mask, need_dx, need_w, affine, fwd_plan.groups, id(fwd_plan))
        plan = self._plans.get(key)
        if plan is None:
            self._cur_groups = fwd_plan.groups
            try:
                plan = self._plans[key] = self._compile_backward(fwd_plan, mode, mask, need_dx, need_w, affine)
            finally:
                self._cur_groups = 1
        self._check_prologue_tables(plan)
        lease = self._arenas.acquire(plan.bscr_bytes, self.device)
        bscr = lease.t
        self._dbg_last = (plan, bscr)
        tensors = {S_X: x, S_P: self._flat_data, S_WP: self._wp, S_ACT: act.t, S_BSCR: bscr, S_OUT0: outs[0]}
        if len(outs) > 1:
            tensors[S_OUT1] = outs[1]
        for slot, d in zip((S_DOUT0, S_DOUT1), douts):
            if d is not None:
                tensors[slot] = d
        dx = gflat = None
        if need_dx:
            dx = self._alloc_out((n, h, w, c))
            tensors[S_DX] = dx
        if need_w:
            gflat = torch.empty(self._pcount, dtype=torch.float32, device=self.device)
            tensors[S_GRAD] = gflat
            self._grad_written = True
            self._grad_is_zero = False
        self._run(plan, tensors)
        return dx, gflat


class MyEncoder(CtlNet):

    def __init__(self, input_channel: int, feature_reduce: int = 4, device="cuda", _spec=None, _prefix="", bf16: bool = False):
        self._px = _prefix
        self.chan = [64 // feature_reduce, 128 // feature_reduce, 256 // feature_reduce, 512 // feature_reduce,
                     512 // feature_reduce]
        super().__init__(_spec if _spec is not None else _init.encoder_spec("", input_channel, feature_reduce),
                         input_channel, device, bf16)

    def _emit_encoder_fwd(self, pb: PlanBuilder, x: T, mode: str, z_out: T):
        C, B, px = self._convs, self._bns, self._px
        train = mode != "C"
        c0, c3 = C[px + "inc.0"], C[px + "inc.3"]
        if c0.wp_c4 >= 0:
            u0, st, blk = pb.conv(x, self._wp_ref(c0.wp_c4), c0.cout, 3, in_mode=_ffi.IN_C4, bias_ref=pb.P(c0.b_off), stats=train)
        else:
            u0, st, blk = pb.conv(x, self._wp_ref(c0.wp_fwd), c0.cout, 3, bias_ref=pb.P(c0.b_off), stats=train)
        co0 = pb.bn_forward(B[px + "inc.1"], st, blk, u0.n * u0.h * u0.w, mode)
        v0, st, blk = pb.conv(u0, self._wp_ref(c3.wp_fwd), c3.cout, 3, pro=(co0["scale"], co0["shift"], SLOPE),
                              bias_ref=pb.P(c3.b_off), stats=train)
        co1 = pb.bn_forward(B[px + "inc.4"], st, blk, v0.n * v0.h * v0.w, mode)
        rec = {"x": x, "u0": u0, "v0": v0, "co0": co0, "co1": co1, "blocks": []}
        cur, cur_pro = v0, (co1["scale"], co1["shift"], SLOPE)
        for i in range(1, 5):
            cur, brec = self._emit_block_fwd(pb, f"{px}down{i}", "down", cur, cur_pro, mode)
            cur_pro = None
            rec["blocks"].append(brec)
        cf = C[px + "final_conv.0"]
        uf, st, blk = pb.conv(cur, self._wp_ref(cf.wp_fwd), cf.cout, 1, bias_ref=pb.P(cf.b_off), stats=train)
        cof = pb.bn_forward(B[px + "final_conv.1"], st, blk, uf.n * uf.h * uf.w, mode)
        pb.bn_act(uf, cof, 0.0, z_out)
        rec.update(uf=uf, cof=cof, z=z_out, x4=cur)
        return rec

    def _emit_encoder_bwd(self, pb: PlanBuilder, rec, dz: T, need_dx: bool, need_w: bool, affine: bool):
        px = self._px
        dbg = {"dz": dz}
        blocks = rec["blocks"]
        tail = self._tail_of(pb, blocks[-1])
        d = self._emit_conv_bn_pair_bwd(pb, px + "final_conv.0", px + "final_conv.1", rec["x4"], None, rec["uf"], rec["cof"], 0.0,
                                        dz, None, need_w, affine, tail_next=tail)
        pre = None
        if tail is not None:
            d, pre = d[0], d[1:]
        dbg["d_down5"] = d
        dbg["tail_down5"] = pre
        u0, v0 = rec["u0"], rec["v0"]
        if pb.b16:
            pair16 = FUSE_PAIR16 and FUSE_BNAPPLY16 and u0.b16 and v0.b16
        else:
            pair16 = FUSE_PAIR and FUSE_BNAPPLY and FUSE_BNBWD and u0.c % 16 == 0
        pair16 = pair16 and pb.groups * u0.c <= 256 and blocks[0].get("drop") is None
        act1 = (v0, rec["co1"]["scale"], rec["co1"]["shift"], SLOPE) if pair16 else None
        act0 = (u0, rec["co0"]["scale"], rec["co0"]["shift"], SLOPE) if pair16 else None
        for i, brec in reversed(list(enumerate(blocks))):
            tail = self._tail_of(pb, blocks[i - 1]) if i >= 1 else None
            d = self._emit_block_bwd(pb, brec, d, None, need_w, affine, pre_tail=pre, tail_next=tail, act_next=act1 if i == 0 else None)
            pre = None
            if tail is not None or (i == 0 and act1 is not None):
                d, pre = d[0], d[1:]
            dbg[f"d_down{i + 1}"] = d
            dbg[f"tail_down{i + 1}"] = pre
        pro0 = (rec["co0"]["scale"], rec["co0"]["shift"], SLOPE)
        d = self._emit_conv_bn_pair_bwd(pb, px + "inc.3", px + "inc.4", u0, pro0, v0, rec["co1"], SLOPE, d, None,
                                        need_w, affine, pre=pre, act_next=act0)
        pre = None
        if act0 is not None:
            d, pre = d[0], d[1:]
        dbg["d_inc3"], dbg["pre_inc3"] = d, pre
        dx = T((S_DX, 0), *rec["x"][1:]) if need_dx else None
        self._emit_conv_bn_pair_bwd(pb, px + "inc.0", px + "inc.1", rec["x"], None, u0, rec["co0"], SLOPE, d, dx,
                                    need_w, affine, need_dx=need_dx, pre=pre)
        return dbg

    def _zdims(self, n, h, w):
        for _ in range(4):
            h, w = (h + 1) // 2, (w + 1) // 2
        return (n, h, w, self.chan[4])

    def _compile_forward(self, n, h, w, mode) -> Plan:
        pb = PlanBuilder(self)
        zs = self._zdims(n, h, w)
        rec = self._emit_encoder_fwd(pb, T((S_X, 0), n, h, w, self.cin), mode, T((S_OUT0, 0), *zs))
        return pb.finish(rec, [zs])

    def _compile_backward(self, fwd: Plan, mode, mask, need_dx, need_w, affine) -> Plan:
        pb = PlanBuilder(self)
        if need_w:
            pb.zero((S_GRAD, 0), 4 * self._pcount)
        z = fwd.rec["z"]
        dbg = self._emit_encoder_bwd(pb, fwd.rec, T((S_DOUT0, 0), *z[1:]), need_dx, need_w, affine)
        return pb.finish(dbg)

    def forward(self, x):
        from .autograd import net_apply
        return net_apply(self, x)[0]


class Dual_Branch_Encoder(MyEncoder):

    def __init__(self, input_channel: int, z_level_1_channel: int = 128, z_level_2_channel: int = 128, feature_reduce: int = 4,
                 device="cuda", bf16: bool = False):
        assert z_level_1_channel == z_level_2_channel == 512 // feature_reduce
        super().__init__(input_channel, feature_reduce, device,
                         _spec=_init.dual_encoder_spec(input_channel, z_level_1_channel, feature_reduce),
                         _prefix="general_encoder.", bf16=bf16)

    def _compile_forward(self, n, h, w, mode) -> Plan:
        pb = PlanBuilder(self)
        C, B = self._convs, self._bns
        train = mode != "C"
        zs = self._zdims(n, h, w)
        z_i, z_s = T((S_OUT0, 0), *zs), T((S_OUT1, 0), *zs)
        rec = self._emit_encoder_fwd(pb, T((S_X, 0), n, h, w, self.cin), mode, z_i)
        d0, d3 = C["code_decoupler.0"], C["code_decoupler.3"]
        ud, st, blk = pb.conv(z_i, self._wp_ref(d0.wp_fwd), d0.cout, 3, bias_ref=pb.P(d0.b_off), stats=train)
        cod0 = pb.bn_forward(B["code_decoupler.1"], st, blk, ud.n * ud.h * ud.w, mode)
        vd, st, blk = pb.conv(ud, self._wp_ref(d3.wp_fwd), d3.cout, 3, pro=(cod0["scale"], cod0["shift"], SLOPE),
                              bias_ref=pb.P(d3.b_off), stats=train)
        cod1 = pb.bn_forward(B["code_decoupler.4"], st, blk, vd.n * vd.h * vd.w, mode)
        pb.bn_act(vd, cod1, 0.0, z_s)
        rec.update(ud=ud, vd=vd, cod0=cod0, cod1=cod1, z_s=z_s)
        return pb.finish(rec, [zs, zs])

    def _compile_backward(self, fwd: Plan, mode, mask, need_dx, need_w, affine) -> Plan:
        pb = PlanBuilder(self)
        rec = fwd.rec
        if need_w:
            pb.zero((S_GRAD, 0), 4 * self._pcount)
        z_i = rec["z"]
        dzi_in = T((S_DOUT0, 0), *z_i[1:]) if mask[0] else None
        extra = {}
        if mask[1]:
            dzs = T((S_DOUT1, 0), *z_i[1:])
            pro = (rec["cod0"]["scale"], rec["cod0"]["shift"], SLOPE)
            d = self._emit_conv_bn_pair_bwd(pb, "code_decoupler.3", "code_decoupler.4", rec["ud"], pro, rec["vd"], rec["cod1"], 0.0,
                                            dzs, None, need_w, affine)
            ci, bn = self._convs["code_decoupler.0"], self._bns["code_decoupler.1"]
            du = pb.bscr.tensor(*rec["ud"][1:])
            pb.bn_backward(1, d, None, rec["ud"], bn, rec["cod0"], SLOPE, ds=None, dx=du, affine_grad=need_w and affine)
            if need_w:
                pb.wgrad(z_i, du, 3, dw_ref=pb.G(ci.w_off), strides=(ci.cin * 9, 9, 3, 1), dbias_ref=pb.G(ci.b_off))
            dzi = pb.bscr.tensor(*z_i[1:], b16=False)
            if dzi_in is not None:
                pb.copy(dzi_in.ref, dzi.ref, 4 * z_i.n * z_i.h * z_i.w * z_i.c)
            pb.conv(du, self._wp_ref(ci.wp_dgrad), ci.cin, 3, out=dzi, accum=dzi_in is not None)
            extra = {"d_cd3": d, "du_cd0": du}
        else:
            dzi = dzi_in
        if dzi is None:
            raise _ffi.CtlError("Dual_Branch_Encoder backward called without any output gradient")
        dbg = self._emit_encoder_bwd(pb, rec, dzi, need_dx, need_w, affine)
        dbg.update(extra)
        return pb.finish(dbg)

    def forward(self, x):
        from .autograd import net_apply
        return net_apply(self, x)

    def _compile_filter(self, n, h, w, mode) -> Plan:
        pb = PlanBuilder(self)
        C, B = self._convs, self._bns
        train = mode != "C"
        d0, d3 = C["code_decoupler.0"], C["code_decoupler.3"]
        z_i, z_s = T((S_X, 0), n, h, w, d0.cin), T((S_OUT0, 0), n, h, w, d3.cout)
        ud, st, blk = pb.conv(z_i, self._wp_ref(d0.wp_fwd), d0.cout, 3, bias_ref=pb.P(d0.b_off), stats=train)
        cod0 = pb.bn_forward(B["code_decoupler.1"], st, blk, ud.n * ud.h * ud.w, mode)
        vd, st, blk = pb.conv(ud, self._wp_ref(d3.wp_fwd), d3.cout, 3, pro=(cod0["scale"], cod0["shift"], SLOPE),
                              bias_ref=pb.P(d3.b_off), stats=train)
        cod1 = pb.bn_forward(B["code_decoupler.4"], st, blk, vd.n * vd.h * vd.w, mode)
        pb.bn_act(vd, cod1, 0.0, z_s)
        return pb.finish({}, [(n, h, w, d3.cout)])

    def filter_code(self, z):
        from . import ops
        ops.require_gpu(z)
        if torch.is_grad_enabled() and z.requires_grad:
            raise _ffi.CtlError("filter_code: forward-only entry (call the encoder's forward for a differentiable z_s)")
        z = ops.as_nhwc(z.detach().float())
        n, c, h, w = z.shape
        d0 = self._convs["code_decoupler.0"]
        if c != d0.cin:
            raise ValueError(f"filter_code: expected {d0.cin} channels, got {c}")
        mode = self.bn_mode()
        key = ("filter", n, h, w, mode)
        plan = self._plans.get(key)
        if plan is None:
            plan = self._plans[key] = self._compile_filter(n, h, w, mode)
        self.ensure_packed()
        act = self._arenas.acquire(plan.act_bytes, self.device)
        out = self._alloc_out(plan.out_shapes[0])
        self._run(plan, {S_X: z, S_P: self._flat_data, S_B: self._bflat, S_NBT: self._nbt, S_WP: self._wp, S_ACT: act.t, S_OUT0: out})
        return out


class MyDecoder(CtlNet):

    def __init__(self, input_channel: int, output_channel: int, feature_reduce: int = 4, up_type: str = "NN",
                 last_act: Optional[str] = None, device="cuda", bf16: bool = False):
        if up_type not in ("NN", "Conv2"):
            raise NotImplementedError(f"up_type {up_type!r} (the reference's FCN_16_standard uses 'NN' and 'Conv2')")
        self.up_type, self.out_ch = up_type, output_channel
        self.sigmoid = last_act in ("sigmoid", "Sigmoid") or isinstance(last_act, nn.Sigmoid)
        super().__init__(_init.decoder_spec(input_channel, output_channel, up_type, feature_reduce), input_channel, device, bf16)

    def _compile_forward(self, n, h, w, mode) -> Plan:
        pb = PlanBuilder(self)
        cur = T((S_X, 0), n, h, w, self.cin)
        rec = {"x": cur, "blocks": []}
        pre = "nn" if self.up_type == "NN" else "convT"
        for i in range(1, 5):
            cur, brec = self._emit_block_fwd(pb, f"up{i}", pre, cur, None, mode)
            rec["blocks"].append(brec)
        cf = self._convs["final_conv"]
        out = T((S_OUT0, 0), cur.n, cur.h, cur.w, cf.cout)
        pb.conv(cur, self._wp_ref(cf.wp_fwd), cf.cout, 1, bias_ref=pb.P(cf.b_off), act=_ffi.ACT_SIGMOID if self.sigmoid else 0,
                out=out)
        rec.update(x4=cur, out=out)
        return pb.finish(rec, [(out.n, out.h, out.w, out.c)])

    def _compile_backward(self, fwd: Plan, mode, mask, need_dx, need_w, affine) -> Plan:
        pb = PlanBuilder(self)
        rec = fwd.rec
        if need_w:
            pb.zero((S_GRAD, 0), 4 * self._pcount)
        out, x4, cf = rec["out"], rec["x4"], self._convs["final_conv"]
        dout = T((S_DOUT0, 0), *out[1:])
        if self.sigmoid:
            dl = pb.bscr.tensor(*out[1:], b16=False)
            pb.sigmoid_bwd(dout, out, dl)
            dout = dl
        if need_w:
            pb.wgrad(x4, dout, 1, dw_ref=pb.G(cf.w_off), strides=(cf.cin, 1, 1, 1), dbias_ref=pb.G(cf.b_off))
        blocks = rec["blocks"]
        tail = self._tail_of(pb, blocks[3])
        d, st, blk = pb.conv(dout, self._wp_ref(cf.wp_dgrad), cf.cin, 1, arena=pb.bscr, tail=tail)
        pre = (st, blk, pb.last_pool) if tail is not None else None
        dbg = {"d_out4": d, "tail_out4": pre}
        for i in range(3, -1, -1):
            d_in = T((S_DX, 0), *rec["x"][1:]) if (i == 0 and need_dx) else None
            tail = self._tail_of(pb, blocks[i - 1]) if i >= 1 else None
            d = self._emit_block_bwd(pb, blocks[i], d, d_in, need_w, affine, pre_tail=pre, tail_next=tail)
            pre = None
            if tail is not None:
                d, pre = d[0], d[1:]
            dbg[f"d_out{i}"] = d
            dbg[f"tail_out{i}"] = pre
        return pb.finish(dbg)

    def forward(self, x):
        from .autograd import net_apply
        return net_apply(self, x)[0]


LABEL_MAXC = 16


def conv_channels_ok(c: int) -> bool:
    return c in (1, 4, 8, 12) or (c >= 16 and c % 16 == 0)


def _internal_widths(reduce_factor: int):
    specs = _init.network_specs(0, 0, reduce_factor)
    return sorted({c for spec in specs.values() for _, kind, a in spec for c in (a[:2] if kind != "bn" else a[:1])} - {0})


def _reduce_factor_ok(rf: int, dtype: str) -> bool:
    w = _internal_widths(rf)
    return 64 // rf >= 1 and all(conv_channels_ok(c) and (dtype != "bf16" or c % 16 == 0) for c in w) and max(w) <= PRO_MAX


def check_config(image_ch: int = 1, num_classes: int = 4, reduce_factor: int = 4, dtype: str = "fp32") -> None:
    if dtype not in ("fp32", "bf16"):
        raise ValueError(f"dtype {dtype!r}: 'fp32' (the reference's arithmetic) or 'bf16' (bf16 storage + MFMA, fp32 accumulate)")
    chans = "1, 4, 8, 12 or a multiple of 16"
    for name, v in (("image_ch", image_ch), ("num_classes", num_classes), ("reduce_factor", reduce_factor)):
        if isinstance(v, bool) or not isinstance(v, (int, np.integer)) or v < 1:
            raise ValueError(f"{name}={v!r}: a positive integer is needed")
    if not conv_channels_ok(image_ch):
        raise ValueError(f"image_ch={image_ch}: the conv kernels take {chans} image channels (pad the images with zero channels to use {image_ch})")
    if not conv_channels_ok(num_classes) or num_classes > LABEL_MAXC:
        ok = [c for c in range(1, LABEL_MAXC + 1) if conv_channels_ok(c)]
        raise ValueError(f"num_classes={num_classes}: accepted are {ok} (conv kernels: {chans}; label-space kernels: at most {LABEL_MAXC} classes)")
    if reduce_factor > 64 or not _reduce_factor_ok(reduce_factor, dtype):
        ok = [r for r in range(1, 65) if _reduce_factor_ok(r, dtype)]
        widths = _internal_widths(reduce_factor) if reduce_factor <= 64 else []
        why = "stores the internal tensors as bf16, in whole 16-channel tiles" if dtype == "bf16" else f"takes internal widths of {chans}"
        why += f", at most {PRO_MAX} wide (the staged BatchNorm coefficient table)"
        raise ValueError(f"reduce_factor={reduce_factor} with dtype={dtype!r}: accepted are {ok} (internal widths {widths}; dtype {dtype!r} {why})")


def build_networks(image_ch: int = 1, num_classes: int = 4, reduce_factor: int = 4, device="cuda",
                   state_dicts: Optional[dict] = None, dtype: str = "fp32", encoder_dropout: Optional[float] = None,
                   decoder_dropout: Optional[float] = None) -> Dict[str, CtlNet]:
    check_config(image_ch, num_classes, reduce_factor, dtype)
    z = 512 // reduce_factor
    sds = state_dicts if state_dicts is not None else _init.reference_init_state_dicts(image_ch, num_classes, reduce_factor)
    b = dtype == "bf16"
    nets = {
        "image_encoder": Dual_Branch_Encoder(image_ch, z, z, reduce_factor, device=device, bf16=b),
        "segmentation_decoder": MyDecoder(z, num_classes, reduce_factor, "NN", None, device=device, bf16=b),
        "shape_encoder": MyEncoder(num_classes, reduce_factor, device=device, bf16=b),
        "shape_decoder": MyDecoder(z, num_classes, reduce_factor, "NN", None, device=device, bf16=b),
        "image_decoder": MyDecoder(z, image_ch, reduce_factor, "Conv2", "sigmoid", device=device, bf16=b),
    }
    for k, net in nets.items():
        if k in sds and sds[k] is not None:
            net.load_state_dict(sds[k])
        net.set_dropout(encoder_dropout if k.endswith("encoder") else decoder_dropout)
    return nets
```

cooperative_training_and_latent_space_data_augmentation_amd/ops.py:

```python
from __future__ import annotations

import ctypes as C
from typing import Optional

import numpy as np
import torch

from . import _ffi
from ._ffi import lib, check


def stream_ptr() -> int:
    return torch.cuda.current_stream().cuda_stream


def ptr(t: Optional[torch.Tensor]) -> Optional[int]:
    return None if t is None else t.data_ptr()


def require_gpu(*ts: torch.Tensor) -> None:
    for t in ts:
        if t is not None and not t.is_cuda:
            raise _ffi.CtlError("the HIP path needs device tensors (got a CPU tensor); there is no CPU fallback")

# ... 268 lines not shown
    masked = torch.empty_like(code)
    mask = torch.empty((n, L), dtype=torch.float32, device=code.device)
    score = torch.empty((n, L), dtype=torch.float32, device=code.device) if want_score else None
    k_dev = k if isinstance(k, torch.Tensor) else None
    k_host = 0 if k_dev is not None else int(k)
    if soft_noise is not None:
        soft_noise = soft_noise.reshape(n, L).float().contiguous()
    need = lib.ctl_latent_mask_fused_ws_floats(mode, n, h * w, c)
    ws = torch.empty(need, dtype=torch.float32, device=code.device) if need else None
    check(lib.ctl_latent_mask_fused(mode, ptr(grad), ptr(code), ptr(soft_noise), k_host, ptr(k_dev), ptr(masked), ptr(mask), ptr(score),
                                    ptr(ws), n, h * w, c, stream_ptr()), "ctl_latent_mask_fused")
    mask = mask.view(n, c, 1, 1) if mode == 0 else mask.view(n, 1, h, w)
    return (masked, mask, score) if want_score else (masked, mask)


def dropout2d(z: torch.Tensor, p: float, keep: Optional[torch.Tensor] = None, seed: int = 0, state: Optional[torch.Tensor] = None,
              want_mask: bool = False):
    require_gpu(z)
    z = as_nhwc(z)
    n, c, h, w = z.shape
    out = torch.empty_like(z)
    keep_out = torch.empty((n, c), dtype=torch.float32, device=z.device)
    mask = torch.empty_like(z) if want_mask else None
    if keep is not None:
        keep = keep.reshape(n, c).float().contiguous()
    check(lib.ctl_dropout2d_ex(ptr(z), ptr(keep), seed & (2 ** 64 - 1), ptr(state), p, ptr(out), ptr(keep_out), ptr(mask), n, h * w, c,
                               stream_ptr()), "ctl_dropout2d_ex")
    return (out, keep_out, mask) if want_mask else (out, keep_out)


def uniform(shape, device, seed: int, state: Optional[torch.Tensor] = None) -> torch.Tensor:
    out = torch.empty(shape, dtype=torch.float32, device=device)
    if state is not None:
        check(lib.ctl_uniform_dev(ptr(out), out.numel(), seed & (2 ** 64 - 1), ptr(state), stream_ptr()), "ctl_uniform_dev")
    else:
        check(lib.ctl_uniform(ptr(out), out.numel(), seed & (2 ** 64 - 1), stream_ptr()), "ctl_uniform")
    return out


def step_tick(state: torch.Tensor) -> None:
    require_gpu(state)
    assert state.dtype == torch.int64 and state.numel() >= 3
    check(lib.ctl_step_tick(ptr(state), stream_ptr()), "ctl_step_tick")


def adam_step(p, g, m, v, lr, beta1, beta2, eps, step, grad_scale=1.0, state: Optional[torch.Tensor] = None):
    require_gpu(p, g, m, v)
    if state is not None:
        check(lib.ctl_adam_dev(ptr(p), ptr(g), ptr(m), ptr(v), p.numel(), lr, beta1, beta2, eps, ptr(state), grad_scale, stream_ptr()),
              "ctl_adam_dev")
    else:
        check(lib.ctl_adam(ptr(p), ptr(g), ptr(m), ptr(v), p.numel(), lr, beta1, beta2, eps, step, grad_scale, stream_ptr()),
              "ctl_adam")


def confusion_hist(label_true: torch.Tensor, label_pred: torch.Tensor, n_class: int, hist: Optional[torch.Tensor] = None) -> torch.Tensor:
    require_gpu(label_true, label_pred)
    lt = label_true.long().contiguous()
    lp = label_pred.to(torch.uint8).contiguous()
    if lt.numel() != lp.numel():
        raise ValueError("confusion_hist: label_true and label_pred differ in size")
    if hist is None:
        hist = torch.zeros((n_class, n_class), dtype=torch.int64, device=lt.device)
    check(lib.ctl_confusion_hist(ptr(lt), ptr(lp), lt.numel(), n_class, ptr(hist), stream_ptr()), "ctl_confusion_hist")
    return hist


def _surface_mode(mode) -> int:
    m = {2: 2, 3: 3, "2d": 2, "3d": 3, "2D": 2, "3D": 3}.get(mode)
    if m is None:
        raise ValueError(f"surface mode {mode!r}: '2d' (every slice on its own) or '3d' (the whole volume)")
    return m


def _surface_sampling(sampling, ndim: int):
    if sampling is None:
        return None
    s = np.ascontiguousarray(np.broadcast_to(np.asarray(sampling, dtype=np.float64), (ndim,)))
    return (C.c_double * ndim)(*s.tolist())


def surface_stats(pred: torch.Tensor, gt: torch.Tensor, n_class: int, sampling=None, connectivity: int = 1, mode="3d",
                  foreground_only: bool = False) -> torch.Tensor:
    require_gpu(pred, gt)
    mode = _surface_mode(mode)
    if pred.dim() != 3 or tuple(pred.shape) != tuple(gt.shape):
        raise ValueError(f"surface_stats: expected two [D,H,W] volumes of one shape, got {tuple(pred.shape)} and {tuple(gt.shape)}")
    p, g = pred.to(torch.uint8).contiguous(), gt.long().contiguous()
    d, h, w = (int(v) for v in p.shape)
    samp = _surface_sampling(sampling, mode)
    rows = lib.ctl_surface_stats_rows(d, n_class, int(foreground_only), mode)
    if rows < 0:
        check(rows, "ctl_surface_stats_rows")
    table = torch.empty((rows, 4), dtype=torch.float64, device=p.device)
    nbytes = lib.ctl_surface_stats_ws_bytes(d, h, w, n_class, int(foreground_only), mode)
    ws = torch.empty(max(nbytes, 1), dtype=torch.uint8, device=p.device)
    check(lib.ctl_surface_stats(ptr(p), ptr(g), d, h, w, n_class, int(foreground_only), mode, int(connectivity), samp, ptr(table), ptr(ws),
                                nbytes, stream_ptr()), "ctl_surface_stats")
    return table.view(-1, 2, d if mode == 2 else 1, 4)


def surface_quantiles(pred: torch.Tensor, gt: torch.Tensor, n_class: int, q=(95.0,), sampling=None, connectivity: int = 1, mode="3d",
                      foreground_only: bool = False, want_stats: bool = False):
    require_gpu(pred, gt)
    mode = _surface_mode(mode)
    if pred.dim() != 3 or tuple(pred.shape) != tuple(gt.shape):
# ... 594 lines not shown
```

cooperative_training_and_latent_space_data_augmentation_amd/optim.py:

```python
from __future__ import annotations

import torch

from . import ops


class FlatAdam:
    def __init__(self, net, lr=1e-4, betas=(0.9, 0.999), eps=1e-8):
        self.net = net
        self.defaults = dict(lr=lr, betas=betas, eps=eps, weight_decay=0, amsgrad=False)
        self.param_groups = [dict(self.defaults, params=list(net.parameters()))]
        self.exp_avg = torch.zeros_like(net._flat_data)
        self.exp_avg_sq = torch.zeros_like(net._flat_data)
        self.step_count = 0

    def zero_grad(self, set_to_none: bool = False):
        self.net.zero_grad()

    def step(self, closure=None, grad_scale: float = 1.0, state=None):
        if not self.net._grad_written:
            return
        g = self.param_groups[0]
        self.step_count += 1
        ops.adam_step(self.net._flat_data, self.net._flat.grad, self.exp_avg, self.exp_avg_sq, g["lr"], g["betas"][0],
                      g["betas"][1], g["eps"], self.step_count, grad_scale, state=state)
        self.net.weights_changed()

    def _views(self, flat):
        net = self.net
        return [flat[net._poff[n]:net._poff[n] + p.numel()].view(p.shape) for n, p in net.named_parameters()]

    def state_dict(self):
        state = {}
        if self.step_count > 0:
            for i, (m, v) in enumerate(zip(self._views(self.exp_avg), self._views(self.exp_avg_sq))):
                state[i] = {"step": torch.tensor(float(self.step_count)), "exp_avg": m.detach().cpu().clone(),
                            "exp_avg_sq": v.detach().cpu().clone()}
        g = {k: v for k, v in self.param_groups[0].items() if k != "params"}
        g["params"] = list(range(len(self.param_groups[0]["params"])))
        return {"state": state, "param_groups": [g]}

    def load_state_dict(self, sd):
        g = sd["param_groups"][0]
        for k in ("lr", "betas", "eps"):
            if k in g:
                self.param_groups[0][k] = tuple(g[k]) if k == "betas" else g[k]
        ms, vs = self._views(self.exp_avg), self._views(self.exp_avg_sq)
        self.step_count = 0
        for i, st in sd["state"].items():
            ms[int(i)].copy_(st["exp_avg"])
            vs[int(i)].copy_(st["exp_avg_sq"])
            self.step_count = int(float(st["step"]))
```

cooperative_training_and_latent_space_data_augmentation_amd/solver.py:

```python
from __future__ import annotations

import gc
import itertools
import os
import random
from os.path import join
from typing import Dict, Optional

import torch
import torch.nn as nn

from . import ops
from .autograd import cross_entropy_2D, net_apply, scaled_mse, segmentation_loss, softmax_t, split_halves
from .losses import parse_loss_type
from .metrics import runningScore
from .model_util import (_disable_tracking_bn_stats, _draw_seed, mask_latent_code_channel_wise,
                         mask_latent_code_spatial_wise, set_grad)
from .nets import build_networks, check_config
from .optim import FlatAdam

_DEFAULT_IMG_CFG = {"loss_name": "mse", "mask_type": "random", "max_threshold": 0.5, "random_threshold": True, "if_soft": True}
_DEFAULT_SEG_CFG = {"loss_name": "ce", "mask_type": "random", "max_threshold": 0.5, "random_threshold": True, "if_soft": True}


def basic_loss_fn(pred, target, loss_type="cross entropy", class_weights=None, use_gpu=True):
    if loss_type == "cross entropy" and class_weights is None:
        return cross_entropy_2D(pred, target)
    terms, class_weights = parse_loss_type(loss_type, class_weights, pred.size(1))
    total = None
    for name, weight in terms:
        l = cross_entropy_2D(pred, target) if name == "cross entropy" else segmentation_loss(pred, target, name, class_weights)
        l = l if weight == 1.0 else l * weight
        total = l if total is None else total + l
    return total


SPLIT_BACKWARD = True
STACK_ALL_FTN = (("image_decoder", 1), ("segmentation_decoder", 0), ("image_encoder", 0))
STACK_PASSES = ()
SPLIT_WGRAD_TAIL = True

class AdvancedTripletReconSegmentationModel(nn.Module):
    def __init__(self, network_type="FCN_16_standard", image_ch=1, learning_rate=1e-4, encoder_dropout=None,
                 decoder_dropout=None, num_classes=4, n_iter=1, checkpoint_dir=None, use_gpu=True, debug=False, *, compute_dtype=None,
                 seg_loss_type="cross entropy", class_weights=None):
        super().__init__()
        self.compute_dtype = compute_dtype or "fp32"
        if network_type not in ("FCN_16_standard", "FCN_16_standard_w_o_filter", "FCN_16_standard_share_code"):
            raise NotImplementedError(network_type)
        if not use_gpu:
            raise RuntimeError("this engine runs on MI355X only (use_gpu=True); the CPU path is the oracle under oracle/")
        check_config(image_ch, num_classes, 4, self.compute_dtype)
        _, class_weights = parse_loss_type(seg_loss_type, class_weights, num_classes)
        self.seg_loss_type = dict(seg_loss_type) if isinstance(seg_loss_type, dict) else seg_loss_type
        self.class_weights = class_weights
        self.network_type, self.image_ch, self.checkpoint_dir = network_type, image_ch, checkpoint_dir
        self.num_classes, self.learning_rate, self.n_iter = num_classes, learning_rate, n_iter
        self.encoder_dropout, self.decoder_dropout = encoder_dropout, decoder_dropout
        self.use_gpu, self.debug = use_gpu, debug
        self.device = torch.device("cuda", torch.cuda.current_device())
        self.model = self.get_network(checkpoint_dir=checkpoint_dir)
        self.optimizers = None
        self.reset_all_optimizers()
        self.latent_code = {"image": None, "segmentation": None, "shape": None}
        self.running_metric = self.set_running_metric()
        self.cur_eval_images = self.cur_eval_predicts = self.cur_eval_gts = None
        self.cur_time_predicts = {}
        self.loss = 0.0
        self.z_i = self.z_s = None
        self.last_masks = {}
        self.grad_scale = 1.0
        self._dp = None
# ... 50 lines not shown

    def save_snapshots(self, save_dir, epoch, model_prefix="interrupted"):
        epoch_path = join(save_dir, "interrupted", "checkpoints")
        os.makedirs(epoch_path, exist_ok=True)
        save_path = join(epoch_path, self.network_type + ".pkl")
        state = {"network_type": self.network_type, "epoch": epoch,
                 "model_state": {k: {n: v.detach().cpu().clone() for n, v in m.state_dict().items()} for k, m in self.model.items()},
                 "optimizer_state": {k: o.state_dict() for k, o in self.optimizers.items()}}
        torch.save(state, save_path)
        return save_path

    def load_snapshots(self, file_path):
        if not file_path or not os.path.exists(file_path):
            print(f"warning: {file_path} does not exists")
            return 0
        ckpt = torch.load(file_path, map_location="cpu")
        for k, net in self.model.items():
            net.load_state_dict(ckpt["model_state"][k])
        for k, opt in self.optimizers.items():
            opt.load_state_dict(ckpt["optimizer_state"][k])
        return ckpt["epoch"]

    def train(self, if_testing=False):
        self.training = True
        for net in self.model.values():
            if not if_testing:
                net.train()
                set_grad(net, True)
            else:
                net.eval()
        return self

    def eval(self):
        self.training = False
        self.train(if_testing=True)
        return self

    def set_optimizers(self):
        self.optimizers = {name: FlatAdam(net, lr=self.learning_rate) for name, net in self.model.items()}

    def reset_all_optimizers(self):
        if self.optimizers is None:
            self.set_optimizers()
        for o in self.optimizers.values():
            o.zero_grad()

    def zero_grad(self):
        self.reset_all_optimizers()

    def get_optimizer(self, model_name=None):
        return self.optimizers if model_name is None else self.optimizers[model_name]

    def optimize_all_params(self):
        for name, o in self.optimizers.items():
            if self._dp is not None:
                self._dp.wait(name)
            o.step(grad_scale=self.grad_scale, state=self._gstate)

    def optimize_params(self, model_name):
        if self._dp is not None:
            self._dp.wait(model_name)
        self.optimizers[model_name].step(grad_scale=self.grad_scale, state=self._gstate)

    def reset_optimizer(self, model_name):
        self.optimizers[model_name].zero_grad()

    def set_running_metric(self):
        return runningScore(n_classes=self.num_classes)

    def get_modules(self):
        return self.model.values()

    def _enc(self, x, disable_track_bn_stats=False):
        enc = self.model["image_encoder"]
        if disable_track_bn_stats:
            with _disable_tracking_bn_stats(enc):
                z_i, z_s = enc(x)
        else:
            z_i, z_s = enc(x)
        if "share_code" in self.network_type:
            z_i = z_s
        elif "w_o_filter" in self.network_type:
            z_s = z_i
        return z_i, z_s

    @staticmethod
    def _call(net, x, disable_track_bn_stats=False):
        if disable_track_bn_stats:
            with _disable_tracking_bn_stats(net):
                return net(x)
        return net(x)

    def encode_image(self, input, disable_track_bn_stats=False):
        z_i, z_s = self._enc(input, disable_track_bn_stats)
        self.latent_code["image"], self.latent_code["segmentation"] = z_i, z_s
        return z_i, z_s

    def decode_image(self, latent_code, disable_track_bn_stats=False):
        return self._call(self.model["image_decoder"], latent_code, disable_track_bn_stats)

    @staticmethod
    def _overlap_probe(a, b, us=300) -> float:
        from .hipgraph import streams_overlap_ratio
        return streams_overlap_ratio(a, b, us)

    def _ensure_chains_overlap(self):
        if torch.cuda.is_current_stream_capturing():
            return
        cur = torch.cuda.current_stream()
# ... 253 lines not shown
            self._join_side()
        finally:
            set_grad(d_seg, requires_grad=True)
            set_grad(d_img, requires_grad=True)
            if gen_corrupted_seg:
                d_seg.forget_pass()
            if gen_corrupted_image:
                d_img.forget_pass()
        return perturbed_image_0, perturbed_y_0

    def slow_refinement(self, pred_logit, n_steps=1, auto_stop=False, save_internal_predicts=False):
        n_steps = self.n_iter if n_steps is None else n_steps
        s_t = pred_logit
        stn_training = self.model["shape_encoder"].training or self.model["shape_decoder"].training
        for _ in range(max(n_steps, 0) if stn_training else min(max(n_steps, 0), 1)):
            s_t = self.recon_shape(pred_logit.detach())
        return s_t, {0: [pred_logit]}

    def predict(self, input, softmax=False, n_iter=None):
        self.eval()
        n_iter = self.n_iter if n_iter is None else n_iter
        with torch.no_grad():
            _, pred = self.fast_predict(input)
            for _ in range(max(n_iter - 1, 0)):
                pred, _ = self.slow_refinement(pred, n_steps=n_iter)
        if softmax:
            pred = softmax_t(pred, 1.0)
        return pred

    def evaluate(self, input, targets_npy, n_iter=None):
        n_iter = self.n_iter if n_iter is None else n_iter
        self.train(if_testing=True)
        pred = self.predict(input, n_iter=n_iter)
        pred_lab = ops.argmax_c(pred)
        if torch.is_tensor(targets_npy) and targets_npy.is_cuda:
            self.running_metric.update(label_trues=targets_npy, label_preds=pred_lab)
            self.cur_eval_images, self.cur_eval_predicts, self.cur_eval_gts = input.detach()[:, 0], pred_lab, targets_npy
            return pred
        pred_npy = pred_lab.cpu().numpy()
        self.running_metric.update(label_trues=targets_npy, label_preds=pred_npy)
        self.cur_eval_images = input.detach().cpu().numpy()[:, 0, :, :]
        self.cur_eval_predicts, self.cur_eval_gts = pred_npy, targets_npy
        return pred

    def get_recon_diff(self, input):
        self.eval()
        with torch.no_grad():
            (z_i, _), first = self.fast_predict(input)
            refined = self.recon_shape(first, is_label_map=False)
            recon = self.decode_image(z_i)
        return torch.abs(input - recon), torch.abs(refined - first), first, refined, recon

    def _two_chain_forward(self, clean_image_l, label_l, image_l, img_cfg, seg_cfg, separate_training, image_override, seg_override):
        for net in self.model.values():
            net.ensure_packed()
        cur, side = torch.cuda.current_stream(), self._side
        self._main = cur
        z_i, z_s = self._enc(image_l)
        self.z_i, self.z_s = z_i, z_s
        if self._chain_events is not None:
            self._fork_event = torch.cuda.Event(enable_timing=True)
            self._fork_event.record(cur)
        side.wait_stream(cur)
        for t in (z_i, z_s, clean_image_l, label_l):
            t.record_stream(side)
        gen_kw = dict(corrupted_image_DA_config=img_cfg, corrupted_seg_DA_config=seg_cfg, image_override=image_override,
                      seg_override=seg_override)
        xh = yh = None
        img_saliency_done = None
        from . import model_util as _mu
        scheme_of = lambda cfg, ov: None if cfg is None else (ov or {}).get("scheme", cfg["mask_type"])
        early_img = _mu.REUSE_SALIENCY_FORWARD and scheme_of(img_cfg, image_override) not in (None, "dropout")
        early_seg = _mu.REUSE_SALIENCY_FORWARD and scheme_of(seg_cfg, seg_override) not in (None, "dropout")
        image_recon_loss = y_0 = None
        if early_img:
            image_recon_loss = scaled_mse(self.decode_image(z_i), clean_image_l, 0.5)
            self._img_std_done = torch.cuda.Event()
            self._img_std_done.record(cur)
            side.wait_event(self._img_std_done)
        if early_seg:
            y_0 = self._call(self.model["segmentation_decoder"], z_s)
        self._in_side = True
        try:
            with torch.cuda.stream(side):
                if img_cfg is not None:
                    xh, _ = self.hard_example_generation(clean_image_l.detach(), label_l.detach(), gen_corrupted_seg=False,
                                                         gen_corrupted_image=True, **gen_kw)
                    if self.last_scheme != "dropout" and not early_img:
                        img_saliency_done = torch.cuda.Event()
                        img_saliency_done.record(side)
        finally:
            self._in_side = False
        if seg_cfg is not None:
            self._in_side = True
            try:
                _, yh = self.hard_example_generation(clean_image_l.detach(), label_l.detach(), gen_corrupted_seg=True,
                                                     gen_corrupted_image=False, **gen_kw)
            finally:
                self._in_side = False
            yh.record_stream(side)
        seg_ready = torch.cuda.Event()
        seg_ready.record(cur)
        if image_recon_loss is None:
            if img_saliency_done is not None:
                cur.wait_event(img_saliency_done)
            image_recon_loss = scaled_mse(self.decode_image(z_i), clean_image_l, 0.5)
            self._img_std_done = torch.cuda.Event()
            self._img_std_done.record(cur)
# ... 130 lines not shown
```

include/ctl_hip.h:

```cpp
#ifndef CTL_HIP_H
#define CTL_HIP_H

#include <stddef.h>
#include <stdint.h>

#ifdef __cplusplus
extern "C" {
#endif

typedef void* ctl_stream;

enum ctl_status { CTL_OK = 0, CTL_EINVAL = -1, CTL_EUNSUPPORTED = -2, CTL_ELAUNCH = -3 };

#define CTL_ABI_VERSION 11
int         ctl_version(void);
const char* ctl_last_error(void);

enum { CTL_IN_PLAIN = 0, CTL_IN_UP2 = 1, CTL_IN_ZINS2 = 2, CTL_IN_C4 = 3  };
enum { CTL_ACT_NONE = 0, CTL_ACT_LEAKY = 1, CTL_ACT_SIGMOID = 2 };
enum { CTL_EPI_BIAS = 1, CTL_EPI_ACCUM = 2, CTL_EPI_RES = 4, CTL_EPI_STATS = 8, CTL_EPI_BNBWD = 16, CTL_EPI_TAILBWD = 32 };

typedef struct ctl_conv {
    int32_t n, hin, win, cin;
    int32_t hout, wout, cout;
// ... 1 lines not shown
    int32_t in_mode;
    int32_t pro_affine;
    float   pro_slope;
    int32_t epi_flags;
    int32_t epi_act;
    float   epi_slope;
    int32_t out_h, out_w;
    int32_t out_sy, out_sx;
    int32_t nsub, out_sub;
    int32_t groups;
    int32_t dt;
} ctl_conv;
enum { CTL_DT_BF16 = 1, CTL_DT_X16 = 2, CTL_DT_Y16 = 4, CTL_DT_RES16 = 8, CTL_DT_X3 = 16 };
enum { CTL_PACK_X3 = 16 };

size_t ctl_conv_wpack_floats(int32_t cin, int32_t cout, int32_t ks);
size_t ctl_conv_stats_floats(const ctl_conv* d);
int    ctl_conv_stats_blocks(const ctl_conv* d);

int ctl_pack_weights(const float* src, float* dst, int32_t cout, int32_t cin, int32_t ks,
                     int64_t s_co, int64_t s_ci, int64_t s_kh, int64_t s_kw, int32_t flip, ctl_stream stream);

int ctl_conv_forward(const ctl_conv* d, const float* x, const float* wpack, const float* bias,
                     const float* pro_scale, const float* pro_shift,
                     const float* res, const float* res_scale, const float* res_shift,
                     float* y, float* stats_partial, ctl_stream stream);
int ctl_conv_forward_ex(const ctl_conv* d, const float* x, const float* wpack, const float* bias,
                        const float* pro_scale, const float* pro_shift,
                        const float* res, const float* res_scale, const float* res_shift, const float* res2, const float* x2,
                        float* y, float* stats_partial, float* pool, float* xout, ctl_stream stream);
int ctl_conv_pool_ok(const ctl_conv* d);

int    ctl_wgrad_splits(const ctl_conv* d);
size_t ctl_wgrad_partial_floats(const ctl_conv* d);
size_t ctl_wgrad_bias_partial_floats(const ctl_conv* d);
int ctl_conv_wgrad(const ctl_conv* d, const float* x, const float* pro_scale, const float* pro_shift,
                   const float* dy, float* w_partial, float* b_partial, ctl_stream stream);
int ctl_conv_wgrad_ex(const ctl_conv* d, const float* x, const float* pro_scale, const float* pro_shift,
                      const float* dy, const float* dy2, const float* dy_coef, float* w_partial, float* b_partial, ctl_stream stream);

int ctl_wgrad_group_class(const ctl_conv* d, int32_t has_dy2);
int ctl_wgrad_group_plan(const ctl_conv* descs, int32_t n, int32_t* splits);
int ctl_conv_wgrad_group(int32_t n, const ctl_conv* descs, const int32_t* splits, const float* const* x, const float* const* pro_scale,
                         const float* const* pro_shift, const float* const* dy, const float* const* dy2, const float* const* dy_coef,
                         float* const* w_partial, float* const* b_partial, ctl_stream stream);
int ctl_wgrad_reduce(const ctl_conv* d, const float* w_partial, const float* b_partial,
                     float* dw, int64_t s_co, int64_t s_ci, int64_t s_kh, int64_t s_kw,
                     float* dbias, int32_t accumulate, ctl_stream stream);

int ctl_pack_weights_batched(const float* params, float* wpack, const int64_t* table, int32_t n_rec, int64_t max_total,
                             ctl_stream stream);
int ctl_wgrad_reduce_batched(const float* scratch, float* grad, const int64_t* table, int32_t n_rec, int64_t max_blocks,
                             ctl_stream stream);
int ctl_pack_weights_bf16_batched(const float* params, float* wpack, const int64_t* table, int32_t n_rec, int64_t max_total,
                                  ctl_stream stream);
size_t ctl_conv_wpack_floats_x3(int32_t cin, int32_t cout, int32_t ks);
int ctl_pack_weights_x3_batched(const float* params, float* wpack, const int64_t* table, int32_t n_rec, int64_t max_total,
                                ctl_stream stream);

int ctl_bn_finalize(const float* partial, int32_t blocks, int32_t c, int64_t count, const float* gamma,
                    const float* beta, float eps, float momentum, int32_t update_running, float* running_mean,
                    float* running_var, int64_t* num_batches_tracked, float* scale, float* shift, float* save_mean,
                    float* save_invstd, int32_t groups, ctl_stream stream);
int ctl_bn_finalize_ex(const float* partial, int32_t blocks, int32_t c, int64_t count, const float* gamma,
                       const float* beta, float eps, float momentum, int32_t update_running, float* running_mean,
                       float* running_var, int64_t* num_batches_tracked, float* scale, float* shift, float* save_mean,
                       float* save_invstd, float* save_uvar, int32_t groups, ctl_stream stream);
int ctl_bn_replay_running(const void* act, float* buffers, int64_t* num_batches_tracked, const int64_t* table, int32_t n_rec,
                          float momentum, ctl_stream stream);
int ctl_bn_eval_coeffs(int32_t c, const float* gamma, const float* beta, const float* running_mean,
                       const float* running_var, float eps, float* scale, float* shift, int32_t groups, ctl_stream stream);
int ctl_bn_act(const float* x, const float* scale, const float* shift, float slope, float* y, int64_t pixels,
               int32_t c, int32_t groups, ctl_stream stream);

#ifndef CTL_RED_BLOCKS
#define CTL_RED_BLOCKS 512
#endif
int ctl_bwd_reduce(int32_t mode, const float* dy, const float* act_src, const float* bn_src, const float* scale,
                   const float* shift, float slope, int64_t pixels, int32_t c, float* partial, int32_t groups,
                   ctl_stream stream);
int ctl_bwd_reduce_rows(int32_t mode, int64_t pixels_per_group, int32_t c);
int ctl_red_blocks(void);
int ctl_bn_bwd_finalize(const float* partial, int32_t c, int64_t count, const float* gamma, const float* save_mean,
                        const float* save_invstd, float* coef, float* dgamma, float* dbeta, int32_t accumulate,
                        int32_t groups, int32_t blocks, ctl_stream stream);
int ctl_bn_bwd_finalize_ex(const float* partial, int32_t c, int64_t count, const float* gamma, const float* save_mean,
                           const float* save_invstd, float* coef, float* dgamma, float* dbeta, int32_t accumulate,
                           int32_t groups, int32_t blocks, uint32_t affine_groups, ctl_stream stream);
int ctl_bwd_apply(int32_t mode, const float* dy, const float* act_src, const float* bn_src, const float* scale,
                  const float* shift, float slope, const float* coef, int64_t pixels, int32_t c, float* ds,
                  float* dx, int32_t groups, ctl_stream stream);
int ctl_chan_sum_finalize(const float* partial, int32_t c, float* out, int32_t accumulate, ctl_stream stream);
int ctl_sumpool2(const float* dup, float* dx, int32_t n, int32_t h, int32_t w, int32_t c, int32_t accumulate,
                 ctl_stream stream);
int ctl_sigmoid_bwd(const float* dy, const float* y, float* dx, int64_t count, ctl_stream stream);

int ctl_softmax_t_fwd(const float* x, float inv_t, float* p, int64_t pixels, int32_t c, ctl_stream stream);
int ctl_softmax_t_bwd(const float* p, const float* dp, float inv_t, float* dx, int64_t pixels, int32_t c,
                      ctl_stream stream);
int ctl_onehot(const int64_t* label, float* y, int64_t pixels, int32_t c, ctl_stream stream);
int ctl_ce2d_fwd(const float* logit, const int64_t* label, int64_t pixels, int32_t c, double* partial, float* loss,
                 ctl_stream stream);
int ctl_ce2d_bwd(const float* logit, const int64_t* label, const float* gout, int64_t pixels, int32_t c,
                 float* dlogit, ctl_stream stream);
enum { CTL_LOSS_WCE = 0, CTL_LOSS_FOCAL = 1, CTL_LOSS_DICE = 2, CTL_LOSS_FG_DICE = 3 };
int32_t ctl_seg_loss_blocks(int32_t b, int64_t hw);
size_t ctl_seg_loss_ws_doubles(int32_t kind, int32_t b, int64_t hw, int32_t c);
int ctl_seg_loss_fwd(int32_t kind, const float* logit, const int64_t* label, const double* class_weights, float gamma, int32_t b,
                     int64_t hw, int32_t c, double* ws, float* loss, ctl_stream stream);
int ctl_seg_loss_bwd(int32_t kind, const float* logit, const int64_t* label, const double* class_weights, float gamma, const float* gout,
                     const double* ws, int32_t b, int64_t hw, int32_t c, float* dlogit, ctl_stream stream);
// ... 74 lines not shown
                  float* field, void* workspace, size_t workspace_bytes, ctl_stream stream);
int ctl_aug_warp(const float* image, const int64_t* label, const float* matrix, const float* intensity, const float* field, int32_t n,
                 int32_t hp, int32_t wp, int32_t hc, int32_t wc, float* image_out, int64_t* label_out, void* workspace,
                 size_t workspace_bytes, ctl_stream stream);
size_t ctl_aug_spline_ws_bytes(int32_t n, int32_t hp, int32_t wp, int32_t n_class);
size_t ctl_aug_warp_cubic_ws_bytes(int32_t n, int32_t hp, int32_t wp, int32_t hc, int32_t wc, int32_t n_class);
int ctl_aug_spline_coeffs(const float* image, const int64_t* label, const float* intensity, int32_t n, int32_t hp, int32_t wp,
                          int32_t n_class, float* coeffs, void* workspace, size_t workspace_bytes, ctl_stream stream);
int ctl_aug_warp_cubic(const float* image, const int64_t* label, const float* matrix, const float* intensity, const float* field, int32_t n,
                       int32_t hp, int32_t wp, int32_t hc, int32_t wc, int32_t n_class, float* image_out, int64_t* label_out,
                       void* workspace, size_t workspace_bytes, ctl_stream stream);
size_t ctl_aug_bias_ws_bytes(int32_t n, int32_t hp, int32_t wp);
int ctl_aug_bias(const float* image, const float* bias, const float* noise, const uint64_t* seeds, int32_t n, int32_t hp, int32_t wp,
                 float* out, void* workspace, size_t workspace_bytes, ctl_stream stream);
int ctl_aug_coarse_field(const float* coarse, int32_t n, int32_t hp, int32_t wp, float* field, ctl_stream stream);

size_t ctl_order_stats_ws_bytes(int32_t segments, int32_t n_rank);
int ctl_order_stats(const float* x, int32_t segments, int64_t seg_elems, const int64_t* ranks, int32_t n_rank, float* out,
                    void* workspace, size_t workspace_bytes, ctl_stream stream);
int ctl_percentile_apply(const float* x, const float* table, int32_t segments, int64_t seg_elems, double g_lo, double g_hi,
                         int32_t form, float new_min, float new_max, float* out, float* bounds, ctl_stream stream);
int ctl_resample_inplane(const float* image, const void* label, int32_t label_bytes, int32_t n, int32_t h, int32_t w, int32_t new_h,
                         int32_t new_w, double r_h, double r_w, float* image_out, void* label_out, ctl_stream stream);

int ctl_restore_scores(const float* scores, int32_t n, int32_t c, int32_t win_h, int32_t win_w, int32_t h, int32_t w, int32_t res_h,
                       int32_t res_w, int32_t off_y, int32_t off_x, double q_h, double q_w, int32_t mode, uint8_t* label, float* soft,
                       ctl_stream stream);
int ctl_restore_labels(const uint8_t* labels, int32_t n, int32_t win_h, int32_t win_w, int32_t h, int32_t w, int32_t res_h, int32_t res_w,
                       int32_t off_y, int32_t off_x, double q_h, double q_w, uint8_t* out, ctl_stream stream);

#define CTL_CORRUPT_MAX_SPIKES 8
#define CTL_CORRUPT_MAX_COPIES 8
#define CTL_CORRUPT_RED_BLOCKS 256
int ctl_corrupt_bias(const float* x, const float* coefficients, int32_t d, int32_t h, int32_t w, float* out, ctl_stream stream);
size_t ctl_corrupt_spike_ws_bytes(int32_t d, int32_t h, int32_t w, int32_t n_spikes);
int ctl_corrupt_spike(const float* x, int32_t d, int32_t h, int32_t w, const int32_t* k, const int32_t* mult, int32_t n_spikes,
                      double intensity, float* out, void* workspace, size_t workspace_bytes, ctl_stream stream);
int ctl_corrupt_rigid3d(const float* x, int32_t d, int32_t h, int32_t w, const float* matrices, int32_t copies, float* out,
                        ctl_stream stream);
int ctl_axis_operator(const float* x0, const float* xs, int32_t n_volumes, int32_t d, int32_t h, int32_t w, int32_t axis,
                      const float* matrix, float* out, ctl_stream stream);

int ctl_slice_foreground(const uint8_t* label, const int64_t* table, int32_t n_slices, int64_t arena_elems, int32_t* counts,
                         ctl_stream stream);
int ctl_batch_gather(const float* image, const uint8_t* label, const int64_t* table, int32_t n_slices, int64_t arena_elems,
                     const int32_t* index, int32_t n, const uint8_t* lut, int32_t H, int32_t W, float* image_out, int64_t* label_out,
                     int32_t Hc, int32_t Wc, float* orig_image, int64_t* orig_label, ctl_stream stream);

int ctl_adam(float* p, const float* g, float* m, float* v, int64_t count, float lr, float beta1, float beta2,
             float eps, int32_t step, float grad_scale, ctl_stream stream);
int ctl_accumulate(float* dst, const float* const* srcs, int32_t k, int64_t count, ctl_stream stream);
int ctl_adam_dev(float* p, const float* g, float* m, float* v, int64_t count, float lr, float beta1, float beta2,
                 float eps, const int64_t* state, float grad_scale, ctl_stream stream);

enum ctl_op_kind {
    CTL_OP_CONV = 1, CTL_OP_WGRAD = 2, CTL_OP_WGRAD_REDUCE = 3, CTL_OP_PACK = 4, CTL_OP_BN_FINALIZE = 5,
    CTL_OP_BN_EVAL = 6, CTL_OP_BN_ACT = 7, CTL_OP_BWD_REDUCE = 8, CTL_OP_BN_BWD_FINALIZE = 9, CTL_OP_BWD_APPLY = 10,
    CTL_OP_CHAN_SUM_FINALIZE = 11, CTL_OP_SUMPOOL2 = 12, CTL_OP_SIGMOID_BWD = 13, CTL_OP_ZERO = 14, CTL_OP_COPY = 15, CTL_OP_PACK_BATCH = 16,
    CTL_OP_WGRAD_REDUCE_BATCH = 17, CTL_OP_DROPOUT2D = 18, CTL_OP_BN_REPLAY = 19,
    CTL_OP_WGRAD_GROUP = 20
};
#define CTL_OP_MAX_T 14
typedef struct ctl_op {
    int32_t kind;
    int32_t i[27];
    float   f[4];
    int32_t slot[CTL_OP_MAX_T];
    int64_t off[CTL_OP_MAX_T];
    int64_t l[4];
} ctl_op;
int ctl_plan_run(const ctl_op* ops, int32_t n_ops, void* const* bases, int32_t n_bases, ctl_stream stream);

int ctl_prof_start(const char* filter);
int ctl_prof_start_sampled(const char* filter, int32_t every);
int ctl_prof_stop(char* out, size_t cap);
unsigned long long ctl_launch_count(void);
size_t ctl_sizeof_op(void);
size_t ctl_sizeof_conv(void);

#ifdef __cplusplus
}
#endif
#endif
```

Measured before the change: 1061.

## Batch Adam updates, weight packing and wgrad reduction across networks into single launches

Adds a multi-record Adam kernel that updates several networks' flat parameters in one launch, a multi-network weight-pack kernel that binary-searches a flattened block table, and a flat wgrad-reduce kernel with no padded grid. The solver calls these instead of per-network launches when data parallelism is off. This is meant to cut kernel launch and Python overhead and remove idle blocks from the padded 2D grids, at the cost of a binary search per block and extra table setup.

```diff
diff --git a/cooperative_training_and_latent_space_data_augmentation_amd/_ffi.py b/cooperative_training_and_latent_space_data_augmentation_amd/_ffi.py
--- a/cooperative_training_and_latent_space_data_augmentation_amd/_ffi.py
+++ b/cooperative_training_and_latent_space_data_augmentation_amd/_ffi.py
@@ -29,6 +29,15 @@
 LOSS_WCE, LOSS_FOCAL, LOSS_DICE, LOSS_FG_DICE = 0, 1, 2, 3
 OP_DTYPE = np.dtype([("kind", "<i4"), ("i", "<i4", (27,)), ("f", "<f4", (4,)), ("slot", "<i4", (OP_MAX_T,)),
                      ("off", "<i8", (OP_MAX_T,)), ("l", "<i8", (4,))], align=True)
+
+
+ADAM_MAX_REC = 8
+PACK_MULTI_WORDS = 16
+
+
+class AdamRec(C.Structure):
+    _fields_ = [("p", C.c_void_p), ("g", C.c_void_p), ("m", C.c_void_p), ("v", C.c_void_p), ("count", C.c_int64),
+                ("lr", C.c_float), ("beta1", C.c_float), ("beta2", C.c_float), ("eps", C.c_float), ("step", C.c_int32)]
 
 
 class CtlError(RuntimeError):
@@ -50,6 +59,7 @@
         lib.ctl_last_error.restype = C.c_char_p
         lib.ctl_version.restype = C.c_int
         lib.ctl_launch_count.restype = C.c_ulonglong
+        lib.ctl_pack_multi_blocks.restype = C.c_int64
         for name in ("ctl_conv_wpack_floats", "ctl_conv_stats_floats", "ctl_wgrad_partial_floats",
                      "ctl_wgrad_bias_partial_floats", "ctl_latent_score_ws_floats", "ctl_latent_mask_apply_ws_floats",
                      "ctl_rescale_intensity_ws_floats", "ctl_sizeof_op", "ctl_sizeof_conv", "ctl_latent_mask_fused_ws_floats", "ctl_conv_wpack_floats_x3",
@@ -108,12 +118,15 @@
             "ctl_uniform_dev": [p, i64, u64, p, p],
             "ctl_adam_dev": [p, p, p, p, i64, f32, f32, f32, f32, p, f32, p],
             "ctl_adam": [p, p, p, p, i64, f32, f32, f32, f32, i32, f32, p],
+            "ctl_adam_multi": [p, i32, p, f32, p],
             "ctl_accumulate": [p, p, i32, i64, p],
             "ctl_plan_run": [p, i32, p, i32, p],
             "ctl_prof_start": [C.c_char_p], "ctl_prof_start_sampled": [C.c_char_p, i32], "ctl_prof_stop": [p, C.c_size_t],
             "ctl_pack_weights_batched": [p, p, p, i32, i64, p], "ctl_wgrad_reduce_batched": [p, p, p, i32, i64, p],
+            "ctl_wgrad_reduce_flat": [p, p, p, i32, i64, p],
             "ctl_pack_weights_bf16_batched": [p, p, p, i32, i64, p],
             "ctl_pack_weights_x3_batched": [p, p, p, i32, i64, p], "ctl_conv_wpack_floats_x3": [i32, i32, i32],
+            "ctl_pack_multi_blocks": [i64, i64], "ctl_pack_weights_multi": [p, i32, i64, p],
             "ctl_bwd_reduce_rows": [i32, i64, i32],
             "ctl_bn_act_dt": [p, p, p, f32, p, i64, i32, i32, C.c_uint32, p],
             "ctl_bwd_reduce_dt": [i32, p, p, p, p, p, f32, i64, i32, p, i32, C.c_uint32, p, p],
@@ -184,7 +197,8 @@
             "ctl_percentile_apply", "ctl_resample_inplane", "ctl_corrupt_bias", "ctl_corrupt_spike_ws_bytes", "ctl_corrupt_spike",
             "ctl_corrupt_rigid3d", "ctl_axis_operator", "ctl_slice_foreground", "ctl_batch_gather", "ctl_surface_quantiles_ws_bytes",
             "ctl_surface_quantiles", "ctl_restore_scores", "ctl_restore_labels", "ctl_seg_loss_blocks", "ctl_seg_loss_ws_doubles",
-            "ctl_seg_loss_fwd", "ctl_seg_loss_bwd"]
+            "ctl_seg_loss_fwd", "ctl_seg_loss_bwd", "ctl_adam_multi", "ctl_pack_multi_blocks", "ctl_pack_weights_multi",
+            "ctl_wgrad_reduce_flat"]
 
 
 def prof_start(kernel_filter: str = "", every: int = 1) -> None:
diff --git a/cooperative_training_and_latent_space_data_augmentation_amd/csrc/ctl_conv.hip b/cooperative_training_and_latent_space_data_augmentation_amd/csrc/ctl_conv.hip
--- a/cooperative_training_and_latent_space_data_augmentation_amd/csrc/ctl_conv.hip
+++ b/cooperative_training_and_latent_space_data_augmentation_amd/csrc/ctl_conv.hip
@@ -616,75 +616,20 @@
     const int64_t total = r[10];
     const int64_t idx = (int64_t)blockIdx.x * blockDim.x + threadIdx.x;
     if (idx >= total || (r[11] & CTL_PACK_X3)) return;
-    const float* src = params + r[0];
-    float* dst = wpack + r[1];
-    const int cout = (int)r[2], cin = (int)r[3], ks = (int)r[4], flip = (int)r[5];
-    const int g_chunks = (cin + 15) / 16;
-    const int j = idx & 3, lane = (idx >> 2) & 63;
-    int64_t rest = idx >> 8;
-    const int g = rest % g_chunks;
-    rest /= g_chunks;
-    const int taps = ks * ks;
-    const int tap = rest % taps;
-    const int cot = rest / taps;
-    const int co = cot * 16 + (lane & 15);
-    const int ci = g * 16 + (lane >> 4) * 4 + j;
-    int kh = tap / ks, kw = tap % ks;
-    float v = 0.f;
-    if (r[11] == 4) {
-        const int c = j, quad = (int)((idx >> 8) % 3), cot4 = (int)((idx >> 8) / 3);
-        const int co4 = cot4 * 16 + (lane & 15), tp = 4 * quad + (lane >> 4);
-        if (co4 < cout && c < cin && tp < 9) v = src[co4 * r[6] + c * r[7] + (tp / 3) * r[8] + (tp % 3) * r[9]];
-        dst[idx] = v;
-        return;
-    }
-    if (r[11] == 1) {
-        if (co < cout && ci < cin) {
-            for (int a = 0; a < 2; ++a) {
-                const int sh = a + 2 - kh;
-                if (sh < 0 || sh > 2) continue;
-                for (int b = 0; b < 2; ++b) {
-                    const int sw = b + 2 - kw;
-                    if (sw < 0 || sw > 2) continue;
-                    v += src[co * r[6] + ci * r[7] + sh * r[8] + sw * r[9]];
-                }
-            }
-        }
-    } else if (r[11] == 2) {
-        if (co < cout && ci < cin) {
-            const int a = flip >> 1, b = flip & 1;
-            const int h0 = (kh == 0) ? 0 : (a ? 2 : 1), h1 = (kh == 0) ? (a ? 1 : 0) : 2;
-            const int w0 = (kw == 0) ? 0 : (b ? 2 : 1), w1 = (kw == 0) ? (b ? 1 : 0) : 2;
-            for (int sh = h0; sh <= h1; ++sh)
-                for (int sw = w0; sw <= w1; ++sw) v += src[co * r[6] + ci * r[7] + sh * r[8] + sw * r[9]];
-        }
-    } else if (r[11] == 3) {
-        if (co < cout && ci < cin) {
-            const int a = flip >> 1, b = flip & 1;
-            const int sh = a ? (kh == 0 ? 2 : 0) : (kh == 0 ? 1 : -1);
-            const int sw = b ? (kw == 0 ? 2 : 0) : (kw == 0 ? 1 : -1);
-            if (sh >= 0 && sw >= 0) v = src[co * r[6] + ci * r[7] + sh * r[8] + sw * r[9]];
-        }
-    } else {
-        if (flip) { kh = ks - 1 - kh; kw = ks - 1 - kw; }
-        if (co < cout && ci < cin) v = src[co * r[6] + ci * r[7] + kh * r[8] + kw * r[9]];
-    }
-    dst[idx] = v;
-}
-
-__global__ __launch_bounds__(256) void wgrad_reduce_batched_kernel(const float* __restrict__ scratch, float* __restrict__ grad,
-                                                                    const int64_t* __restrict__ table) {
-    __shared__ float sm[32][65];
-    const int64_t* r = table + (int64_t)blockIdx.y * 16;
+    pack_fp32_element(params, wpack, r, idx);
+}
+
+__device__ __forceinline__ void wgrad_reduce_record(const float* __restrict__ scratch, float* __restrict__ grad, const int64_t* __restrict__ r,
+                                                    int64_t bx, float (*sm)[65]) {
     const int splits = (int)r[4], taps = (int)(r[5] & 0xff), ks = (int)(r[5] >> 8), cin = (int)r[6], cout = (int)r[7];
     const int cin_p = (int)r[8], cout_p = (int)r[9];
     const int64_t total = (int64_t)taps * cin * cout;
     const bool has_b = r[1] >= 0 && r[3] >= 0;
     const bool wide = splits <= 64;
     const int EW = wide ? 64 : 8, SLN = wide ? 4 : 32;
-    if ((int64_t)blockIdx.x * EW >= total + (has_b ? cout : 0)) return;
+    if (bx * EW >= total + (has_b ? cout : 0)) return;
     const int e = wide ? (threadIdx.x & 63) : (threadIdx.x & 7), sl = wide ? (threadIdx.x >> 6) : (threadIdx.x >> 3);
-    const int64_t idx = (int64_t)blockIdx.x * EW + e;
+    const int64_t idx = bx * EW + e;
     const bool is_w = idx < total, is_b = !is_w && has_b && idx < total + cout;
     float v = 0.f;
     int co = 0, ci = 0, tap = 0;
@@ -715,6 +660,22 @@
         *dst = r[14] ? (*dst + t) : t;
     }
 }
+__global__ __launch_bounds__(256) void wgrad_reduce_batched_kernel(const float* __restrict__ scratch, float* __restrict__ grad,
+                                                                    const int64_t* __restrict__ table) {
+    __shared__ float sm[32][65];
+    wgrad_reduce_record(scratch, grad, table + (int64_t)blockIdx.y * 16, (int64_t)blockIdx.x, sm);
+}
+__global__ __launch_bounds__(256) void wgrad_reduce_flat_kernel(const float* __restrict__ scratch, float* __restrict__ grad,
+                                                                 const int64_t* __restrict__ table, int n_rec) {
+    __shared__ float sm[32][65];
+    int lo = 0, hi = n_rec - 1;
+    while (lo < hi) {
+        const int mid = (lo + hi + 1) >> 1;
+        if ((int64_t)blockIdx.x >= table[(int64_t)mid * 16 + 15]) lo = mid; else hi = mid - 1;
+    }
+    const int64_t* r = table + (int64_t)lo * 16;
+    wgrad_reduce_record(scratch, grad, r, (int64_t)blockIdx.x - r[15], sm);
+}
 
 extern "C" int ctl_pack_weights_batched(const float* params, float* wpack, const int64_t* table, int32_t n_rec,
                                         int64_t max_total, ctl_stream stream) {
@@ -722,6 +683,13 @@
     pack_weights_batched_kernel<<<dim3((unsigned)ctl_cdiv64(max_total, 256), (unsigned)n_rec), dim3(256), 0, (hipStream_t)stream>>>(
         params, wpack, table);
     CTL_LAUNCH_CHECK("pack_weights_batched");
+    return CTL_OK;
+}
+extern "C" int ctl_wgrad_reduce_flat(const float* scratch, float* grad, const int64_t* table, int32_t n_rec, int64_t blocks,
+                                     ctl_stream stream) {
+    CTL_REQUIRE(scratch && grad && table && n_rec > 0 && blocks > 0 && blocks <= 0x7fffffff, "wgrad_reduce_flat: bad arguments");
+    wgrad_reduce_flat_kernel<<<dim3((unsigned)blocks), dim3(256), 0, (hipStream_t)stream>>>(scratch, grad, table, n_rec);
+    CTL_LAUNCH_CHECK("wgrad_reduce_flat");
     return CTL_OK;
 }
 extern "C" int ctl_wgrad_reduce_batched(const float* scratch, float* grad, const int64_t* table, int32_t n_rec,
diff --git a/cooperative_training_and_latent_space_data_augmentation_amd/csrc/ctl_conv_common.h b/cooperative_training_and_latent_space_data_augmentation_amd/csrc/ctl_conv_common.h
--- a/cooperative_training_and_latent_space_data_augmentation_amd/csrc/ctl_conv_common.h
+++ b/cooperative_training_and_latent_space_data_augmentation_amd/csrc/ctl_conv_common.h
@@ -63,3 +63,61 @@
         n += dn;
     }
 };
+
+__device__ __forceinline__ void pack_fp32_element(const float* __restrict__ params, float* __restrict__ wpack, const int64_t* __restrict__ r,
+                                                  int64_t idx) {
+    const float* src = params + r[0];
+    float* dst = wpack + r[1];
+    const int cout = (int)r[2], cin = (int)r[3], ks = (int)r[4], flip = (int)r[5];
+    const int g_chunks = (cin + 15) / 16;
+    const int j = idx & 3, lane = (idx >> 2) & 63;
+    int64_t rest = idx >> 8;
+    const int g = rest % g_chunks;
+    rest /= g_chunks;
+    const int taps = ks * ks;
+    const int tap = rest % taps;
+    const int cot = rest / taps;
+    const int co = cot * 16 + (lane & 15);
+    const int ci = g * 16 + (lane >> 4) * 4 + j;
+    int kh = tap / ks, kw = tap % ks;
+    float v = 0.f;
+    if (r[11] == 4) {
+        const int c = j, quad = (int)((idx >> 8) % 3), cot4 = (int)((idx >> 8) / 3);
+        const int co4 = cot4 * 16 + (lane & 15), tp = 4 * quad + (lane >> 4);
+        if (co4 < cout && c < cin && tp < 9) v = src[co4 * r[6] + c * r[7] + (tp / 3) * r[8] + (tp % 3) * r[9]];
+        dst[idx] = v;
+        return;
+    }
+    if (r[11] == 1) {
+        if (co < cout && ci < cin) {
+            for (int a = 0; a < 2; ++a) {
+                const int sh = a + 2 - kh;
+                if (sh < 0 || sh > 2) continue;
+                for (int b = 0; b < 2; ++b) {
+                    const int sw = b + 2 - kw;
+                    if (sw < 0 || sw > 2) continue;
+                    v += src[co * r[6] + ci * r[7] + sh * r[8] + sw * r[9]];
+                }
+            }
+        }
+    } else if (r[11] == 2) {
+        if (co < cout && ci < cin) {
+            const int a = flip >> 1, b = flip & 1;
+            const int h0 = (kh == 0) ? 0 : (a ? 2 : 1), h1 = (kh == 0) ? (a ? 1 : 0) : 2;
+            const int w0 = (kw == 0) ? 0 : (b ? 2 : 1), w1 = (kw == 0) ? (b ? 1 : 0) : 2;
+            for (int sh = h0; sh <= h1; ++sh)
+                for (int sw = w0; sw <= w1; ++sw) v += src[co * r[6] + ci * r[7] + sh * r[8] + sw * r[9]];
+        }
+    } else if (r[11] == 3) {
+        if (co < cout && ci < cin) {
+            const int a = flip >> 1, b = flip & 1;
+            const int sh = a ? (kh == 0 ? 2 : 0) : (kh == 0 ? 1 : -1);
+            const int sw = b ? (kw == 0 ? 2 : 0) : (kw == 0 ? 1 : -1);
+            if (sh >= 0 && sw >= 0) v = src[co * r[6] + ci * r[7] + sh * r[8] + sw * r[9]];
+        }
+    } else {
+        if (flip) { kh = ks - 1 - kh; kw = ks - 1 - kw; }
+        if (co < cout && ci < cin) v = src[co * r[6] + ci * r[7] + kh * r[8] + kw * r[9]];
+    }
+    dst[idx] = v;
+}
diff --git a/cooperative_training_and_latent_space_data_augmentation_amd/csrc/ctl_conv_x3.hip b/cooperative_training_and_latent_space_data_augmentation_amd/csrc/ctl_conv_x3.hip
--- a/cooperative_training_and_latent_space_data_augmentation_amd/csrc/ctl_conv_x3.hip
+++ b/cooperative_training_and_latent_space_data_augmentation_amd/csrc/ctl_conv_x3.hip
@@ -60,14 +60,12 @@
     }
     return v;
 }
-__global__ void pack_weights_x3_batched_kernel(const float* __restrict__ params, float* __restrict__ wpack, const int64_t* __restrict__ table) {
-    const int64_t* r = table + (int64_t)blockIdx.y * 12;
-    if (!(r[11] & CTL_PACK_X3)) return;
+__device__ __forceinline__ void pack_x3_element(const float* __restrict__ params, float* __restrict__ wpack, const int64_t* __restrict__ r,
+                                                int64_t idx) {
     const int mode = (int)(r[11] & ~(int64_t)CTL_PACK_X3);
     const int cout = (int)r[2], cin = (int)r[3], ks = (int)r[4];
     const int g_chunks = (cin + 15) / 16, taps = ks * ks, nfrag = (taps + 1) / 2;
     const int64_t total = (int64_t)((cout + 15) / 16) * nfrag * g_chunks * 64 * 4;
-    const int64_t idx = (int64_t)blockIdx.x * blockDim.x + threadIdx.x;
     if (idx >= total) return;
     const float* src = params + r[0];
     unsigned* dst = reinterpret_cast<unsigned*>(wpack + r[1]);
@@ -89,6 +87,26 @@
 #pragma unroll
     for (int sp = 0; sp < 3; ++sp) dst[base + sp * 256] = x3_pack2(x3_part(a, sp), x3_part(b, sp));
 }
+__global__ void pack_weights_x3_batched_kernel(const float* __restrict__ params, float* __restrict__ wpack, const int64_t* __restrict__ table) {
+    const int64_t* r = table + (int64_t)blockIdx.y * 12;
+    if (!(r[11] & CTL_PACK_X3)) return;
+    pack_x3_element(params, wpack, r, (int64_t)blockIdx.x * blockDim.x + threadIdx.x);
+}
+__global__ __launch_bounds__(256) void pack_weights_multi_kernel(const int64_t* __restrict__ table, int n_rec) {
+    int lo = 0, hi = n_rec - 1;
+    while (lo < hi) {
+        const int mid = (lo + hi + 1) >> 1;
+        if ((int64_t)blockIdx.x >= table[(int64_t)mid * CTL_PACK_MULTI_WORDS + 14]) lo = mid; else hi = mid - 1;
+    }
+    const int64_t* r = table + (int64_t)lo * CTL_PACK_MULTI_WORDS;
+    const int64_t lb = (int64_t)blockIdx.x - r[14];
+    if (lb >= r[15]) return;
+    const float* params = reinterpret_cast<const float*>((uintptr_t)r[12]);
+    float* wpack = reinterpret_cast<float*>((uintptr_t)r[13]);
+    const int64_t idx = lb * 256 + threadIdx.x;
+    if (r[11] & CTL_PACK_X3) pack_x3_element(params, wpack, r, idx);
+    else if (idx < r[10]) pack_fp32_element(params, wpack, r, idx);
+}
 extern "C" size_t ctl_conv_wpack_floats_x3(int32_t cin, int32_t cout, int32_t ks) {
     return (size_t)ctl_cdiv(cout, 16) * ((ks * ks + 1) / 2) * ctl_cdiv(cin, 16) * 3 * 256;
 }
@@ -96,6 +114,17 @@
     CTL_REQUIRE(params && wpack && table && n_rec > 0 && max_total > 0, "pack_weights_x3_batched: bad arguments");
     pack_weights_x3_batched_kernel<<<dim3((unsigned)ctl_cdiv64(max_total, 3 * 256) + 1, (unsigned)n_rec), dim3(256), 0, (hipStream_t)stream>>>(params, wpack, table);
     CTL_LAUNCH_CHECK("pack_weights_x3_batched");
+    return CTL_OK;
+}
+
+extern "C" int64_t ctl_pack_multi_blocks(int64_t total, int64_t mode) {
+    if (total <= 0) return -1;
+    return ctl_cdiv64((mode & CTL_PACK_X3) ? total / 3 : total, 256);
+}
+extern "C" int ctl_pack_weights_multi(const int64_t* table, int32_t n_rec, int64_t blocks, ctl_stream stream) {
+    CTL_REQUIRE(table && n_rec > 0 && blocks > 0 && blocks <= 0x7fffffff, "pack_weights_multi: bad arguments");
+    pack_weights_multi_kernel<<<dim3((unsigned)blocks), dim3(256), 0, (hipStream_t)stream>>>(table, n_rec);
+    CTL_LAUNCH_CHECK("pack_weights_multi");
     return CTL_OK;
 }
 
diff --git a/cooperative_training_and_latent_space_data_augmentation_amd/csrc/ctl_elem.hip b/cooperative_training_and_latent_space_data_augmentation_amd/csrc/ctl_elem.hip
--- a/cooperative_training_and_latent_space_data_augmentation_amd/csrc/ctl_elem.hip
+++ b/cooperative_training_and_latent_space_data_augmentation_amd/csrc/ctl_elem.hip
@@ -587,18 +587,27 @@
     }
 }
 
-__global__ __launch_bounds__(EB) void adam_kernel(float* __restrict__ p, const float* __restrict__ g, float* __restrict__ m,
-                                                   float* __restrict__ v, int64_t count, float lr, float b1, float b2,
-                                                   float eps, float bc1, float bc2_sqrt, float gscale,
-                                                   const int64_t* __restrict__ state) {
+struct adam_rec_dev { float* p; const float* g; float* m; float* v; int64_t count; float lr, b1, b2, eps, bc1, bc2_sqrt; unsigned blk0, nblk; };
+struct adam_args { adam_rec_dev r[CTL_ADAM_MAX_REC]; };
+__global__ __launch_bounds__(EB) void adam_kernel(adam_args a, int n_rec, float gscale, const int64_t* __restrict__ state) {
+    int ri = 0;
+    for (int k = 1; k < n_rec; ++k)
+        if (blockIdx.x >= a.r[k].blk0) ri = k;
+    float* __restrict__ p = a.r[ri].p;
+    const float* __restrict__ g = a.r[ri].g;
+    float* __restrict__ m = a.r[ri].m;
+    float* __restrict__ v = a.r[ri].v;
+    const int64_t count = a.r[ri].count;
+    const float lr = a.r[ri].lr, b1 = a.r[ri].b1, b2 = a.r[ri].b2, eps = a.r[ri].eps;
+    float bc1 = a.r[ri].bc1, bc2_sqrt = a.r[ri].bc2_sqrt;
     if (state) {
         const double st = (double)state[2];
         bc1 = (float)(1.0 - pow((double)b1, st));
         bc2_sqrt = (float)sqrt(1.0 - pow((double)b2, st));
     }
-    const int64_t stride = (int64_t)gridDim.x * EB;
+    const int64_t stride = (int64_t)a.r[ri].nblk * EB;
     const float step_size = lr / bc1;
-    for (int64_t i = (int64_t)blockIdx.x * EB + threadIdx.x; i < count; i += stride) {
+    for (int64_t i = (int64_t)(blockIdx.x - a.r[ri].blk0) * EB + threadIdx.x; i < count; i += stride) {
         const float gi = g[i] * gscale;
         const float mi = b1 * m[i] + (1.f - b1) * gi;
         const float vi = b2 * v[i] + (1.f - b2) * gi * gi;
@@ -886,20 +895,43 @@
     CTL_LAUNCH_CHECK("argmax_c");
     return CTL_OK;
 }
+static int adam_launch(const ctl_adam_rec* recs, int n_rec, bool dev, float grad_scale, const int64_t* state, hipStream_t s) {
+    adam_args a;
+    unsigned blocks = 0;
+    for (int k = 0; k < CTL_ADAM_MAX_REC; ++k) {
+        adam_rec_dev& d = a.r[k];
+        if (k >= n_rec) { d = adam_rec_dev{nullptr, nullptr, nullptr, nullptr, 0, 0.f, 0.f, 0.f, 0.f, 1.f, 1.f, blocks, 0u}; continue; }
+        const ctl_adam_rec& r = recs[k];
+        const double bc1 = dev ? 1.0 : 1.0 - pow((double)r.beta1, (double)r.step);
+        const double bc2 = dev ? 1.0 : 1.0 - pow((double)r.beta2, (double)r.step);
+        d = adam_rec_dev{r.p, r.g, r.m, r.v, r.count, r.lr, r.beta1, r.beta2, r.eps, (float)bc1, (float)sqrt(bc2), blocks, stream_blocks(r.count)};
+        blocks += d.nblk;
+    }
+    adam_kernel<<<dim3(blocks), dim3(EB), 0, s>>>(a, n_rec, grad_scale, state);
+    return 0;
+}
 extern "C" int ctl_adam(float* p, const float* g, float* m, float* v, int64_t count, float lr, float beta1, float beta2,
                         float eps, int32_t step, float grad_scale, ctl_stream stream) {
     CTL_REQUIRE(p && g && m && v && count > 0 && step >= 1, "adam: bad arguments");
-    const double bc1 = 1.0 - pow((double)beta1, (double)step);
-    const double bc2 = 1.0 - pow((double)beta2, (double)step);
-    adam_kernel<<<dim3(stream_blocks(count)), dim3(EB), 0, S_>>>(p, g, m, v, count, lr, beta1, beta2, eps, (float)bc1,
-                                                                 (float)sqrt(bc2), grad_scale, nullptr);
+    const ctl_adam_rec r{p, g, m, v, count, lr, beta1, beta2, eps, step};
+    adam_launch(&r, 1, false, grad_scale, nullptr, S_);
     CTL_LAUNCH_CHECK("adam");
     return CTL_OK;
 }
 extern "C" int ctl_adam_dev(float* p, const float* g, float* m, float* v, int64_t count, float lr, float beta1, float beta2,
                             float eps, const int64_t* state, float grad_scale, ctl_stream stream) {
     CTL_REQUIRE(p && g && m && v && count > 0 && state, "adam_dev: bad arguments");
-    adam_kernel<<<dim3(stream_blocks(count)), dim3(EB), 0, S_>>>(p, g, m, v, count, lr, beta1, beta2, eps, 1.f, 1.f, grad_scale, state);
+    const ctl_adam_rec r{p, g, m, v, count, lr, beta1, beta2, eps, 0};
+    adam_launch(&r, 1, true, grad_scale, state, S_);
     CTL_LAUNCH_CHECK("adam_dev");
     return CTL_OK;
 }
+extern "C" int ctl_adam_multi(const ctl_adam_rec* recs, int32_t n_rec, const int64_t* state, float grad_scale, ctl_stream stream) {
+    CTL_REQUIRE(recs && n_rec >= 1 && n_rec <= CTL_ADAM_MAX_REC, "adam_multi: bad arguments (1 <= n_rec <= %d)", CTL_ADAM_MAX_REC);
+    for (int k = 0; k < n_rec; ++k)
+        CTL_REQUIRE(recs[k].p && recs[k].g && recs[k].m && recs[k].v && recs[k].count > 0 && (state || recs[k].step >= 1),
+                    "adam_multi: bad record %d", k);
+    adam_launch(recs, n_rec, state != nullptr, grad_scale, state, S_);
+    CTL_LAUNCH_CHECK("adam_multi");
+    return CTL_OK;
+}
diff --git a/cooperative_training_and_latent_space_data_augmentation_amd/csrc/ctl_plan.cpp b/cooperative_training_and_latent_space_data_augmentation_amd/csrc/ctl_plan.cpp
--- a/cooperative_training_and_latent_space_data_augmentation_amd/csrc/ctl_plan.cpp
+++ b/cooperative_training_and_latent_space_data_augmentation_amd/csrc/ctl_plan.cpp
@@ -309,7 +309,8 @@
                 if (rc == CTL_OK && (op.i[1] & 2)) rc = ctl_pack_weights_x3_batched(CF(0), F(1), (const int64_t*)t[2], op.i[0], op.l[0], stream);
                 break;
             case CTL_OP_WGRAD_REDUCE_BATCH:
-                rc = ctl_wgrad_reduce_batched(CF(0), F(1), (const int64_t*)t[2], op.i[0], op.l[0], stream);
+                rc = op.i[1] ? ctl_wgrad_reduce_flat(CF(0), F(1), (const int64_t*)t[2], op.i[0], op.l[0], stream)
+                             : ctl_wgrad_reduce_batched(CF(0), F(1), (const int64_t*)t[2], op.i[0], op.l[0], stream);
                 break;
             case CTL_OP_DROPOUT2D:
                 rc = ctl_dropout2d_dt(t[0], CF(1), (uint64_t)op.l[0], (const int64_t*)t[2], op.f[0], t[3], F(4), op.i[0], op.i[1], op.i[2], (uint32_t)op.i[25], stream);
diff --git a/cooperative_training_and_latent_space_data_augmentation_amd/nets.py b/cooperative_training_and_latent_space_data_augmentation_amd/nets.py
--- a/cooperative_training_and_latent_space_data_augmentation_amd/nets.py
+++ b/cooperative_training_and_latent_space_data_augmentation_amd/nets.py
@@ -204,6 +204,7 @@
         self.table: Optional[np.ndarray] = None
         self.bn_log: List[tuple] = []
         self.pro_entries = 0
+        self.grad_cover: Optional[np.ndarray] = None
 
     def op(self, kind: int) -> np.ndarray:
         r = np.zeros((), dtype=OP_DTYPE)
@@ -346,6 +347,13 @@
         self.reduce_recs.append([wref[1] // 4, bref[1] // 4 if bref else -1, dw_ref[1] // 4, dbias_ref[1] // 4 if dbias_ref else -1,
                                  splits, (ks * ks) | (ks << 8), cin, cout, cin_p, cout_p, *[int(v) for v in strides],
                                  1 if accumulate else 0, 0])
+        if self.grad_cover is not None:
+            assert not accumulate, "a plan without a gradient fill has no accumulating writer"
+            s_co, s_ci, s_kh, s_kw = (int(v) for v in strides)
+            k = np.arange(ks)
+            self._covers(dw_ref, (np.arange(cout) * s_co)[:, None, None, None] + (np.arange(cin) * s_ci)[None, :, None, None] +
+                         (k * s_kh)[None, None, :, None] + (k * s_kw)[None, None, None, :])
+            self._covers(dbias_ref, np.arange(cout))
 
     def flush_wgrad_groups(self):
         pend, self.pending_wgrads = self.pending_wgrads, []
@@ -371,12 +379,23 @@
     def flush_wgrad_reductions(self):
         self.flush_wgrad_groups()
         if not self.reduce_recs:
+            assert self.grad_cover is None, "a backward plan with parameter gradients has weight-gradient reductions"
             return
         assert self.table is None
+        if self.grad_cover is not None:
+            gaps = np.flatnonzero(np.diff(np.concatenate(([False], ~self.grad_cover, [False])).astype(np.int8)))
+            for a, b in zip(gaps[0::2], gaps[1::2]):
+                n = int(b) - int(a)
+                self.reduce_recs.append([-1, -1, int(a), -1, 0, 1 | (1 << 8), 1, n, 16, _rup(n, 16), 1, 0, 0, 0, 0, 0])
+            self.grad_cover = None
+        first = 0
+        for r in self.reduce_recs:
+            r[15] = first
+            first += -(-((r[5] & 0xff) * r[6] * r[7] + (r[7] if r[1] >= 0 and r[3] >= 0 else 0)) // (64 if r[4] <= 64 else 8))
         self.table = np.asarray(self.reduce_recs, dtype=np.int64)
         op = self.op(_ffi.OP_WGRAD_REDUCE_BATCH)
-        op["i"][0] = len(self.reduce_recs)
-        op["l"][0] = max(-(-((r[5] & 0xff) * r[6] * r[7] + r[7]) // (64 if r[4] <= 64 else 8)) for r in self.reduce_recs)
+        op["i"][0], op["i"][1] = len(self.reduce_recs), 1
+        op["l"][0] = first
         self.set_t(op, 0, (S_BSCR, 0))
         self.set_t(op, 1, (S_GRAD, 0))
         self.set_t(op, 2, (S_TAB, 0))
@@ -440,6 +459,9 @@
         for idx, ref in enumerate([part, self.P(bn.g_off), co["mean"], co["invstd"], coef,
                                    self.G(bn.g_off) if affine_grad else None, self.G(bn.b_off) if affine_grad else None]):
             self.set_t(op, idx, ref)
+        if affine_grad:
+            self._covers(self.G(bn.g_off), np.arange(c))
+            self._covers(self.G(bn.b_off), np.arange(c))
         if dx is None:
             return coef
         op = self.op(_ffi.OP_BWD_APPLY)
@@ -468,6 +490,9 @@
         for idx, ref in enumerate([stats_ref, self.P(bn.g_off), co["mean"], co["invstd"], coef,
                                    self.G(bn.g_off) if affine_grad else None, self.G(bn.b_off) if affine_grad else None]):
             self.set_t(op, idx, ref)
+        if affine_grad:
+            self._covers(self.G(bn.g_off), np.arange(c))
+            self._covers(self.G(bn.b_off), np.arange(c))
         if dx is None:
             return coef
         op = self.op(_ffi.OP_BWD_APPLY)
@@ -491,6 +516,7 @@
         op["i"][0], op["i"][1] = c, 0
         self.set_t(op, 0, part)
         self.set_t(op, 1, out_ref)
+        self._covers(out_ref, np.arange(c))
 
     def sumpool2(self, dup: T, dx: T, accumulate=False):
         op = self.op(_ffi.OP_SUMPOOL2)
@@ -514,6 +540,16 @@
         op["l"][0] = salt
         for idx, ref in enumerate([z.ref, keep_in, None if keep_in is not None else (S_STATE, 0), out.ref, keep_out]):
             self.set_t(op, idx, ref)
+
+    def clear_grad(self, count):
+        if self.split_tail:
+            self.zero((S_GRAD, 0), 4 * count)
+        else:
+            self.grad_cover = np.zeros(count, dtype=bool)
+
+    def _covers(self, ref, idx):
+        if self.grad_cover is not None and ref is not None and ref[0] == S_GRAD:
+            self.grad_cover[ref[1] // 4 + np.asarray(idx).ravel()] = True
 
     def zero(self, ref, nbytes):
         op = self.op(_ffi.OP_ZERO)
@@ -1254,7 +1290,7 @@
             self._run(plan, tensors, ops=plan.tail_ops)
         return dx, gflat
 
-    def run_backward(self, x, act, outs, fwd_plan: Plan, mode: str, douts, need_dx: bool, need_w: bool, affine: bool):
+    def run_backward(self, x, act, outs, fwd_plan: Plan, mode: str, douts, need_dx: bool, need_w: bool, affine: bool, grad_out=None):
         n, c, h, w = x.shape
         mask = tuple(d is not None for d in douts)
         key = ("b", n, h, w, mode, mask, need_dx, need_w, affine, fwd_plan.groups, id(fwd_plan))
@@ -1280,7 +1316,8 @@
             dx = self._alloc_out((n, h, w, c))
             tensors[S_DX] = dx
         if need_w:
-            gflat = torch.empty(self._pcount, dtype=torch.float32, device=self.device)
+            gflat = grad_out if grad_out is not None else torch.empty(self._pcount, dtype=torch.float32, device=self.device)
+            assert gflat.numel() == self._pcount and gflat.dtype == torch.float32 and gflat.is_contiguous()
             tensors[S_GRAD] = gflat
             self._grad_written = True
             self._grad_is_zero = False
@@ -1376,7 +1413,7 @@
     def _compile_backward(self, fwd: Plan, mode, mask, need_dx, need_w, affine) -> Plan:
         pb = PlanBuilder(self)
         if need_w:
-            pb.zero((S_GRAD, 0), 4 * self._pcount)
+            pb.clear_grad(self._pcount)
         z = fwd.rec["z"]
         dbg = self._emit_encoder_bwd(pb, fwd.rec, T((S_DOUT0, 0), *z[1:]), need_dx, need_w, affine)
         return pb.finish(dbg)
@@ -1416,7 +1453,7 @@
         pb = PlanBuilder(self)
         rec = fwd.rec
         if need_w:
-            pb.zero((S_GRAD, 0), 4 * self._pcount)
+            pb.clear_grad(self._pcount)
         z_i = rec["z"]
         dzi_in = T((S_DOUT0, 0), *z_i[1:]) if mask[0] else None
         extra = {}
@@ -1512,7 +1549,7 @@
         pb = PlanBuilder(self)
         rec = fwd.rec
         if need_w:
-            pb.zero((S_GRAD, 0), 4 * self._pcount)
+            pb.clear_grad(self._pcount)
         out, x4, cf = rec["out"], rec["x4"], self._convs["final_conv"]
         dout = T((S_DOUT0, 0), *out[1:])
         if self.sigmoid:
@@ -1579,6 +1616,47 @@
         raise ValueError(f"reduce_factor={reduce_factor} with dtype={dtype!r}: accepted are {ok} (internal widths {widths}; dtype {dtype!r} {why})")
 
 
+class _MultiPack:
+    __slots__ = ("plans", "ptrs", "table", "n_rec", "blocks")
+
+    def __init__(self, nets):
+        self.plans = [n._pack_plan for n in nets]
+        self.ptrs = [(n._flat_data.data_ptr(), n._wp.data_ptr()) for n in nets]
+        rows, blocks = [], 0
+        for n, (pp, wp) in zip(nets, self.ptrs):
+            for r in n._pack_plan.table_np.reshape(-1, 12):
+                nb = int(lib.ctl_pack_multi_blocks(int(r[10]), int(r[11])))
+                rows.append([*(int(v) for v in r), pp, wp, blocks, nb])
+                blocks += nb
+        self.table = torch.from_numpy(np.asarray(rows, dtype=np.int64)).to(nets[0].device)
+        self.n_rec, self.blocks = len(rows), blocks
+
+    def matches(self, nets) -> bool:
+        return len(nets) == len(self.plans) and all(n._pack_plan is pl and (n._flat_data.data_ptr(), n._wp.data_ptr()) == pt
+                                                    for n, pl, pt in zip(nets, self.plans, self.ptrs))
+
+
+def ensure_packed_all(nets):
+    nets = list(nets)
+    group = [n for n in nets if not n.bf16]
+    for n in nets:
+        if n.bf16:
+            n.ensure_packed()
+    if not group:
+        return
+    if not group[0]._flat_data.is_cuda:
+        raise _ffi.CtlError("the HIP engine needs the network on a GPU device; there is no CPU fallback")
+    mp = group[0].__dict__.get("_multi_pack")
+    if mp is None or not mp.matches(group):
+        mp = group[0].__dict__["_multi_pack"] = _MultiPack(group)
+    if all(n._packed_ok for n in group):
+        return
+    check(lib.ctl_pack_weights_multi(mp.table.data_ptr(), mp.n_rec, mp.blocks, torch.cuda.current_stream().cuda_stream),
+          "ctl_pack_weights_multi")
+    for n in group:
+        n._packed_ok = True
+
+
 def build_networks(image_ch: int = 1, num_classes: int = 4, reduce_factor: int = 4, device="cuda",
                    state_dicts: Optional[dict] = None, dtype: str = "fp32", encoder_dropout: Optional[float] = None,
                    decoder_dropout: Optional[float] = None) -> Dict[str, CtlNet]:
diff --git a/cooperative_training_and_latent_space_data_augmentation_amd/ops.py b/cooperative_training_and_latent_space_data_augmentation_amd/ops.py
--- a/cooperative_training_and_latent_space_data_augmentation_amd/ops.py
+++ b/cooperative_training_and_latent_space_data_augmentation_amd/ops.py
@@ -344,6 +344,15 @@
     else:
         check(lib.ctl_adam(ptr(p), ptr(g), ptr(m), ptr(v), p.numel(), lr, beta1, beta2, eps, step, grad_scale, stream_ptr()),
               "ctl_adam")
+
+
+def adam_step_multi(records, grad_scale=1.0, state: Optional[torch.Tensor] = None):
+    require_gpu(*[t for r in records for t in r[:4]])
+    arr = (_ffi.AdamRec * len(records))()
+    for a, (p, g, m, v, lr, b1, b2, eps, step) in zip(arr, records):
+        a.p, a.g, a.m, a.v, a.count = ptr(p), ptr(g), ptr(m), ptr(v), p.numel()
+        a.lr, a.beta1, a.beta2, a.eps, a.step = lr, b1, b2, eps, int(step)
+    check(lib.ctl_adam_multi(arr, len(records), ptr(state), grad_scale, stream_ptr()), "ctl_adam_multi")
 
 
 def confusion_hist(label_true: torch.Tensor, label_pred: torch.Tensor, n_class: int, hist: Optional[torch.Tensor] = None) -> torch.Tensor:
diff --git a/cooperative_training_and_latent_space_data_augmentation_amd/optim.py b/cooperative_training_and_latent_space_data_augmentation_amd/optim.py
--- a/cooperative_training_and_latent_space_data_augmentation_amd/optim.py
+++ b/cooperative_training_and_latent_space_data_augmentation_amd/optim.py
@@ -2,7 +2,7 @@
 
 import torch
 
-from . import ops
+from . import _ffi, ops
 
 
 class FlatAdam:
@@ -25,6 +25,11 @@
         ops.adam_step(self.net._flat_data, self.net._flat.grad, self.exp_avg, self.exp_avg_sq, g["lr"], g["betas"][0],
                       g["betas"][1], g["eps"], self.step_count, grad_scale, state=state)
         self.net.weights_changed()
+
+    def _record(self):
+        g = self.param_groups[0]
+        return (self.net._flat_data, self.net._flat.grad, self.exp_avg, self.exp_avg_sq, g["lr"], g["betas"][0], g["betas"][1], g["eps"],
+                self.step_count)
 
     def _views(self, flat):
         net = self.net
@@ -51,3 +56,14 @@
             ms[int(i)].copy_(st["exp_avg"])
             vs[int(i)].copy_(st["exp_avg_sq"])
             self.step_count = int(float(st["step"]))
+
+
+def step_all(optimizers, grad_scale: float = 1.0, state=None):
+    todo = [o for o in optimizers if o.net._grad_written]
+    for i in range(0, len(todo), _ffi.ADAM_MAX_REC):
+        chunk = todo[i:i + _ffi.ADAM_MAX_REC]
+        for o in chunk:
+            o.step_count += 1
+        ops.adam_step_multi([o._record() for o in chunk], grad_scale, state=state)
+        for o in chunk:
+            o.net.weights_changed()
diff --git a/cooperative_training_and_latent_space_data_augmentation_amd/solver.py b/cooperative_training_and_latent_space_data_augmentation_amd/solver.py
--- a/cooperative_training_and_latent_space_data_augmentation_amd/solver.py
+++ b/cooperative_training_and_latent_space_data_augmentation_amd/solver.py
@@ -16,8 +16,8 @@
 from .metrics import runningScore
 from .model_util import (_disable_tracking_bn_stats, _draw_seed, mask_latent_code_channel_wise,
                          mask_latent_code_spatial_wise, set_grad)
-from .nets import build_networks, check_config
-from .optim import FlatAdam
+from .nets import build_networks, check_config, ensure_packed_all
+from .optim import FlatAdam, step_all
 
 _DEFAULT_IMG_CFG = {"loss_name": "mse", "mask_type": "random", "max_threshold": 0.5, "random_threshold": True, "if_soft": True}
 _DEFAULT_SEG_CFG = {"loss_name": "ce", "mask_type": "random", "max_threshold": 0.5, "random_threshold": True, "if_soft": True}
@@ -174,9 +174,11 @@
         return self.optimizers if model_name is None else self.optimizers[model_name]
 
     def optimize_all_params(self):
+        if self._dp is None:
+            step_all(self.optimizers.values(), grad_scale=self.grad_scale, state=self._gstate)
+            return
         for name, o in self.optimizers.items():
-            if self._dp is not None:
-                self._dp.wait(name)
+            self._dp.wait(name)
             o.step(grad_scale=self.grad_scale, state=self._gstate)
 
     def optimize_params(self, model_name):
@@ -536,8 +538,7 @@
         return torch.abs(input - recon), torch.abs(refined - first), first, refined, recon
 
     def _two_chain_forward(self, clean_image_l, label_l, image_l, img_cfg, seg_cfg, separate_training, image_override, seg_override):
-        for net in self.model.values():
-            net.ensure_packed()
+        ensure_packed_all(self.model.values())
         cur, side = torch.cuda.current_stream(), self._side
         self._main = cur
         z_i, z_s = self._enc(image_l)
diff --git a/include/ctl_hip.h b/include/ctl_hip.h
--- a/include/ctl_hip.h
+++ b/include/ctl_hip.h
@@ -77,11 +77,15 @@
                              ctl_stream stream);
 int ctl_wgrad_reduce_batched(const float* scratch, float* grad, const int64_t* table, int32_t n_rec, int64_t max_blocks,
                              ctl_stream stream);
+int ctl_wgrad_reduce_flat(const float* scratch, float* grad, const int64_t* table, int32_t n_rec, int64_t blocks, ctl_stream stream);
 int ctl_pack_weights_bf16_batched(const float* params, float* wpack, const int64_t* table, int32_t n_rec, int64_t max_total,
                                   ctl_stream stream);
 size_t ctl_conv_wpack_floats_x3(int32_t cin, int32_t cout, int32_t ks);
 int ctl_pack_weights_x3_batched(const float* params, float* wpack, const int64_t* table, int32_t n_rec, int64_t max_total,
                                 ctl_stream stream);
+#define CTL_PACK_MULTI_WORDS 16
+int64_t ctl_pack_multi_blocks(int64_t total, int64_t mode);
+int ctl_pack_weights_multi(const int64_t* table, int32_t n_rec, int64_t blocks, ctl_stream stream);
 
 int ctl_bn_finalize(const float* partial, int32_t blocks, int32_t c, int64_t count, const float* gamma,
                     const float* beta, float eps, float momentum, int32_t update_running, float* running_mean,
@@ -262,6 +266,14 @@
 int ctl_accumulate(float* dst, const float* const* srcs, int32_t k, int64_t count, ctl_stream stream);
 int ctl_adam_dev(float* p, const float* g, float* m, float* v, int64_t count, float lr, float beta1, float beta2,
                  float eps, const int64_t* state, float grad_scale, ctl_stream stream);
+#define CTL_ADAM_MAX_REC 8
+typedef struct ctl_adam_rec {
+    float* p; const float* g; float* m; float* v;
+    int64_t count;
+    float lr, beta1, beta2, eps;
+    int32_t step;
+} ctl_adam_rec;
+int ctl_adam_multi(const ctl_adam_rec* recs, int32_t n_rec, const int64_t* state, float grad_scale, ctl_stream stream);
 
 enum ctl_op_kind {
     CTL_OP_CONV = 1, CTL_OP_WGRAD = 2, CTL_OP_WGRAD_REDUCE = 3, CTL_OP_PACK = 4, CTL_OP_BN_FINALIZE = 5,
```

Result: no change. 1060 (-0.1%).
